# lightonai/fast-plaid

Measured on NVIDIA H100. Metric: queries/sec @ top_k=100, 1M-doc/128-dim index; MaxSim HBM GB/s vs roofline, higher is better.
Workload: dtype f16

## Files before the change

fast_plaid_b200/csrc/common.cuh:

```cuda
#pragma once

#include <cuda_fp16.h>
#include <cuda_runtime.h>
#include <stdint.h>

#include "../../include/fastplaid_b200.h"

struct WPerm {
  uint16_t v[16];
};

struct fpb_index {
  int device;
  int nbits;
  int dim;
  int pd;
  int sm_count;
  int64_t K;
  int64_t N;
  int64_t E;
  int64_t n_ivf;
  int64_t max_doc_len;
  int64_t doc_id_base;
  const __half* centroids;
  const int64_t* doc_offsets;
  const int32_t* doc_codes;
  const uint8_t* doc_residuals;
  const __half* token_norms;
  const int64_t* ivf_offsets;
  const int32_t* ivf_pids;
  WPerm w_perm;
  alignas(64) unsigned char tmap_centroids[128];
  int has_tmap;
};

void fpb_set_error(const char* fmt, ...);

#define FPB_CUDA_CHECK(expr)                                                              \
  do {                                                                                    \
    cudaError_t _e = (expr);                                                              \
    if (_e != cudaSuccess) {                                                              \
      fpb_set_error("%s failed: %s (%s:%d)", #expr, cudaGetErrorString(_e), __FILE__, __LINE__); \
      return FPB_ERR_CUDA;                                                                \
    }                                                                                     \
  } while (0)

#define FPB_LAUNCH_CHECK(name)                                                            \
  do {                                                                                    \
    cudaError_t _e = cudaGetLastError();                                                  \
    if (_e != cudaSuccess) {                                                              \
      fpb_set_error("launch of %s failed: %s", name, cudaGetErrorString(_e));            \
      return FPB_ERR_CUDA;                                                                \
    }                                                                                     \
  } while (0)

static inline int64_t fpb_align256(int64_t x) { return (x + 255) & ~int64_t(255); }
static inline int fpb_next_pow2(int x) {
  int p = 1;
  while (p < x) p <<= 1;
  return p;
}


__device__ __forceinline__ uint32_t f32_key(float f) {
  uint32_t u = __float_as_uint(f);
  if ((u << 1) == 0u) u = 0u;
  return (u & 0x80000000u) ? ~u : (u | 0x80000000u);
}
__device__ __forceinline__ float f32_unkey(uint32_t k) {
  uint32_t u = (k & 0x80000000u) ? (k & 0x7fffffffu) : ~k;
  return __uint_as_float(u);
}
__device__ __forceinline__ uint32_t f16_key(uint16_t h) {
  uint32_t u = h;
  if ((u & 0x7fffu) == 0u) u = 0u;
  return (u & 0x8000u) ? (~u & 0xffffu) : (u | 0x8000u);
}

__device__ __forceinline__ uint4 ldg_nc_na(const uint4* p) {
  uint4 r;
  asm volatile("ld.global.nc.L1::no_allocate.v4.u32 {%0,%1,%2,%3}, [%4];"
               : "=r"(r.x), "=r"(r.y), "=r"(r.z), "=r"(r.w)
               : "l"(p));
  return r;
}

__device__ __forceinline__ uint32_t smem_u32(const void* p) {
  return static_cast<uint32_t>(__cvta_generic_to_shared(p));
}

__device__ __forceinline__ void ldmatrix_x4(uint32_t& r0, uint32_t& r1, uint32_t& r2, uint32_t& r3,
                                            uint32_t addr) {
  asm volatile("ldmatrix.sync.aligned.m8n8.x4.shared.b16 {%0,%1,%2,%3}, [%4];"
               : "=r"(r0), "=r"(r1), "=r"(r2), "=r"(r3)
               : "r"(addr));
}

__device__ __forceinline__ void mma_16816(float (&c)[4], const uint32_t (&a)[4], uint32_t b0,
                                          uint32_t b1) {
  asm volatile(
      "mma.sync.aligned.m16n8k16.row.col.f32.f16.f16.f32 {%0,%1,%2,%3}, {%4,%5,%6,%7}, {%8,%9}, "
      "{%0,%1,%2,%3};"
      : "+f"(c[0]), "+f"(c[1]), "+f"(c[2]), "+f"(c[3])
      : "r"(a[0]), "r"(a[1]), "r"(a[2]), "r"(a[3]), "r"(b0), "r"(b1));
}

__device__ __forceinline__ uint32_t pack_half2_rn(float lo, float hi) {
  __half2 h = __floats2half2_rn(lo, hi);
  return *reinterpret_cast<uint32_t*>(&h);
}
__device__ __forceinline__ __half2 u32_as_half2(uint32_t u) { return *reinterpret_cast<__half2*>(&u); }
__device__ __forceinline__ uint32_t half2_as_u32(__half2 h) { return *reinterpret_cast<uint32_t*>(&h); }

#define FPB_PAD_SENTINEL (-10000.0f)
```

fast_plaid_b200/csrc/index.cu:

```cuda
#include <stdarg.h>
#include <stdio.h>
#include <string.h>

#include <cuda.h>

#include "kernels.h"

typedef CUresult (*fpb_encode_tiled_fn)(CUtensorMap*, CUtensorMapDataType, cuuint32_t, void*, const cuuint64_t*,
                                        const cuuint64_t*, const cuuint32_t*, const cuuint32_t*,
                                        CUtensorMapInterleave, CUtensorMapSwizzle, CUtensorMapL2promotion,
                                        CUtensorMapFloatOOBfill);

static int make_centroid_tmap(fpb_index* ix) {
  ix->has_tmap = 0;
  if (ix->dim != 128) return 0;
  void* fn = nullptr;
  cudaDriverEntryPointQueryResult qres;
  if (cudaGetDriverEntryPoint("cuTensorMapEncodeTiled", &fn, cudaEnableDefault, &qres) != cudaSuccess || !fn ||
      qres != cudaDriverEntryPointSuccess) {
    cudaGetLastError();
    return 0;
  }
  static_assert(sizeof(CUtensorMap) == 128, "CUtensorMap is 128 bytes");
  CUtensorMap* tm = reinterpret_cast<CUtensorMap*>(ix->tmap_centroids);
  const cuuint64_t gdim[2] = {cuuint64_t(ix->dim), cuuint64_t(ix->K)};
  const cuuint64_t gstride[1] = {cuuint64_t(ix->dim) * 2};
  const cuuint32_t box[2] = {64, 128};
  const cuuint32_t estr[2] = {1, 1};
  const CUresult r = reinterpret_cast<fpb_encode_tiled_fn>(fn)(
      tm, CU_TENSOR_MAP_DATA_TYPE_FLOAT16, 2, const_cast<__half*>(ix->centroids), gdim, gstride, box, estr,
      CU_TENSOR_MAP_INTERLEAVE_NONE, CU_TENSOR_MAP_SWIZZLE_128B, CU_TENSOR_MAP_L2_PROMOTION_L2_256B,
      CU_TENSOR_MAP_FLOAT_OOB_FILL_NONE);
  if (r == CUDA_SUCCESS) ix->has_tmap = 1;
  return 0;
}

static thread_local char g_err[512] = "";

void fpb_set_error(const char* fmt, ...) {
  va_list ap;
  va_start(ap, fmt);
  vsnprintf(g_err, sizeof(g_err), fmt, ap);
  va_end(ap);
}

extern "C" const char* fpb_last_error(void) { return g_err; }
extern "C" int fpb_abi_version(void) { return 6; }

static int bitrev(int x, int nbits) {
  int r = 0;
  for (int k = 0; k < nbits; ++k)
    if (x & (1 << k)) r |= 1 << (nbits - 1 - k);
  return r;
}

extern "C" int fpb_index_create(fpb_index** out, int device, int nbits, int dim, int64_t n_centroids,
                                const void* d_centroids, const void* d_bucket_weights,
                                int64_t n_docs, const int64_t* d_doc_offsets,
                                const int32_t* d_doc_codes, const uint8_t* d_doc_residuals, void* d_token_norms,
                                const int64_t* d_ivf_offsets, const int32_t* d_ivf_pids,
                                int64_t n_ivf, int64_t max_doc_len, int64_t doc_id_base) {
  if (!out) {
    fpb_set_error("fpb_index_create: out is NULL");
    return FPB_ERR_INVALID;
  }
  *out = nullptr;
  if (nbits != 2 && nbits != 4) {
    fpb_set_error("unsupported nbits=%d (2 and 4 are supported)", nbits);
    return FPB_ERR_UNSUPPORTED;
  }
  const int pd = dim * nbits / 8;
  if ((dim != 64 && dim != 128) || (pd != 16 && pd != 32 && pd != 64)) {
    fpb_set_error("unsupported embedding dim=%d with nbits=%d: this build supports dim 64 and 128", dim, nbits);
    return FPB_ERR_UNSUPPORTED;
  }
  if (n_centroids <= 0 || n_docs < 0 || !d_centroids || !d_bucket_weights || !d_doc_offsets) {
    fpb_set_error("fpb_index_create: bad sizes or NULL codec/offset pointers");
    return FPB_ERR_INVALID;
  }
  if (n_docs >= (int64_t(1) << 31) || n_centroids >= (int64_t(1) << 31)) {
    fpb_set_error("fpb_index_create: n_docs and n_centroids must fit in int32 per shard");
    return FPB_ERR_UNSUPPORTED;
  }
  FPB_CUDA_CHECK(cudaSetDevice(device));
  fpb_index* ix = new fpb_index();
  memset(ix, 0, sizeof(*ix));
  ix->device = device;
  ix->nbits = nbits;
  ix->dim = dim;
  ix->pd = pd;
  ix->K = n_centroids;
  ix->N = n_docs;
  ix->n_ivf = n_ivf;
  ix->max_doc_len = max_doc_len;
  ix->doc_id_base = doc_id_base;
  ix->centroids = static_cast<const __half*>(d_centroids);
  ix->doc_offsets = d_doc_offsets;
  ix->doc_codes = d_doc_codes;
  ix->doc_residuals = d_doc_residuals;
  ix->token_norms = static_cast<const __half*>(d_token_norms);
  ix->ivf_offsets = d_ivf_offsets;
  ix->ivf_pids = d_ivf_pids;
  cudaDeviceProp prop;
  cudaError_t e = cudaGetDeviceProperties(&prop, device);
  if (e != cudaSuccess) {
    delete ix;
    fpb_set_error("cudaGetDeviceProperties failed: %s", cudaGetErrorString(e));
    return FPB_ERR_CUDA;
  }
  ix->sm_count = prop.multiProcessorCount;
  uint16_t w[16];
  e = cudaMemcpy(w, d_bucket_weights, sizeof(uint16_t) * (1 << nbits), cudaMemcpyDeviceToHost);
  if (e != cudaSuccess) {
    delete ix;
    fpb_set_error("copy of bucket_weights failed: %s", cudaGetErrorString(e));
    return FPB_ERR_CUDA;
  }
  for (int i = 0; i < 16; ++i) ix->w_perm.v[i] = 0;
  for (int i = 0; i < (1 << nbits); ++i) ix->w_perm.v[i] = w[bitrev(i, nbits)];
  int64_t n_tokens = 0;
  if (n_docs > 0) {
    e = cudaMemcpy(&n_tokens, d_doc_offsets + n_docs, sizeof(int64_t), cudaMemcpyDeviceToHost);
    if (e != cudaSuccess) {
      delete ix;
      fpb_set_error("copy of doc_offsets[N] failed: %s", cudaGetErrorString(e));
      return FPB_ERR_CUDA;
    }
  }
  ix->E = n_tokens;
  if (n_tokens > 0 && !d_token_norms) {
    delete ix;
    fpb_set_error("fpb_index_create: d_token_norms (f16 [n_tokens], filled here) is NULL");
    return FPB_ERR_INVALID;
  }
  if (n_tokens > 0) {
    const int rc = launch_token_norms(ix, static_cast<__half*>(d_token_norms), nullptr);
    e = rc == FPB_OK ? cudaDeviceSynchronize() : cudaSuccess;
    if (rc != FPB_OK || e != cudaSuccess) {
      delete ix;
      if (rc == FPB_OK) fpb_set_error("token norm kernel failed: %s", cudaGetErrorString(e));
      return rc != FPB_OK ? rc : FPB_ERR_CUDA;
    }
  }
  make_centroid_tmap(ix);
  *out = ix;
  return FPB_OK;
}

extern "C" void fpb_index_destroy(fpb_index* index) { delete index; }

extern "C" int fpb_workspace_layout(const fpb_index* ix, int B, int Q, const fpb_params* p,
                                    fpb_layout* L) {
  if (!ix || !p || !L) {
    fpb_set_error("fpb_workspace_layout: NULL argument");
    return FPB_ERR_INVALID;
  }
  if (B <= 0 || Q <= 0) {
    fpb_set_error("fpb_workspace_layout: B=%d Q=%d must be positive", B, Q);
    return FPB_ERR_INVALID;
  }
  if (Q > 256) {
    fpb_set_error("queries with more than 256 tokens are not supported (Q=%d)", Q);
    return FPB_ERR_UNSUPPORTED;
  }
  if (p->n_ivf_probe < 1 || p->n_ivf_probe > 32) {
    fpb_set_error("n_ivf_probe=%d outside the supported range [1,32]", p->n_ivf_probe);
    return FPB_ERR_UNSUPPORTED;
  }
  if (p->n_full_scores < 1 || p->top_k < 1) {
    fpb_set_error("n_full_scores and top_k must be >= 1");
    return FPB_ERR_INVALID;
  }
  int R = p->n_full_scores / 4;
  if (R < 1) R = 1;
  if (R > 4096) {
    fpb_set_error("n_full_scores=%d: more than 4096 re-ranked documents per query is not supported",
                  p->n_full_scores);
    return FPB_ERR_UNSUPPORTED;
  }
  memset(L, 0, sizeof(*L));
  int Qp = fpb_next_pow2(Q < 16 ? 16 : Q);
  L->B = B;
  L->Q = Q;
  L->Qp = Qp;
  L->n_tiles = int((ix->K + 127) / 128);
  L->R = R;
  L->n_probe = p->n_ivf_probe;
  L->cand_cap = int(ix->N > 0 ? ix->N : 1);
  L->bitmap_words = int((ix->N + 31) / 32) + 1;
  int64_t off = 0;
  auto take = [&](int64_t bytes) {
    int64_t o = off;
    off += fpb_align256(bytes);
    return o;
  };
  L->off_queries = take(int64_t(B) * Qp * ix->dim * 2);
  L->off_S = take(int64_t(B) * ix->K * Qp * 2);
  L->off_tmax = take(int64_t(B) * Qp * L->n_tiles * 2);
  L->off_cells = take(int64_t(B) * Q * L->n_probe * 4);
  L->off_bitmap = take(int64_t(B) * L->bitmap_words * 4);
  L->off_n_cand = take(int64_t(B) * 4);
  L->off_cand = take(int64_t(B) * L->cand_cap * 4);
  L->off_approx = take(int64_t(B) * L->cand_cap * 4);
  L->off_work = take(int64_t(B + 8) * 4);
  L->off_n_rerank = take(int64_t(B) * 4);
  L->off_rerank = take(int64_t(B) * R * 4);
  L->off_rerank_approx = take(int64_t(B) * R * 4);
  L->off_exact = take(int64_t(B) * R * 4);
  const bool sub = (p->flags & FPB_FLAG_SUBSET) != 0;
  L->cbitmap_words = int((ix->K + 31) / 32) + 1;
  L->off_cbitmap = take(sub ? int64_t(B) * L->cbitmap_words * 4 : 0);
  L->off_clist = take(sub ? int64_t(B) * ix->K * 4 : 0);
  L->off_n_clist = take(sub ? int64_t(B) * 4 : 0);
  L->off_sbitmap = take(sub ? int64_t(B) * L->bitmap_words * 4 : 0);
  const bool direct = (p->flags & FPB_FLAG_APPROX_DIRECT) != 0;
  L->hb_words = int(((ix->K + 31) / 32 + 3) / 4 * 4);
  L->off_tau = take(direct ? 0 : int64_t(B) * Qp * 2);
  L->off_hibits = take(direct ? 0 : int64_t(B) * L->hb_words * 4);
  L->off_lb = take(direct ? 0 : int64_t(B) * L->cand_cap * 4);
  L->off_refine = take(direct ? 0 : int64_t(B) * L->cand_cap * 4);
  L->off_n_refine = take(int64_t(B) * 4);
  L->off_thresh = take(int64_t(B) * 4);
  L->off_work2 = take(int64_t(B + 8) * 4);
  L->off_stats = take(8 * 8);
  L->flags = p->flags;
  L->total_bytes = off;
  return FPB_OK;
}
```

fast_plaid_b200/csrc/k3_approx.cu:

```cuda
#include <math.h>
#include <stdlib.h>

#include "kernels.h"

namespace {

constexpr int64_t K3_TWO_PASS_MIN_TOKENS = 200000000;
constexpr int K3_THREADS = 256;
constexpr int K3_DOCS_PER_CHUNK = 64;
constexpr int K3A_DOCS_PER_CHUNK = 128;
constexpr int K3_WQ_FOR(int W, int FLUSH) { int n = 64; while (n < 32 * W + FLUSH) n <<= 1; return n; }

__global__ void k3_prefix_kernel(const int32_t* __restrict__ n_items, int B, int per_chunk,
                                 int32_t* __restrict__ work) {
  if (threadIdx.x == 0 && blockIdx.x == 0) {
    int acc = 0;
    for (int b = 0; b < B; ++b) {
      work[b] = acc;
      acc += (n_items[b] + per_chunk - 1) / per_chunk;
    }
    work[B] = acc;
    work[B + 1] = 0;
  }
}

__device__ __forceinline__ void k3_next_chunk(int32_t* work, int B, int* s_b, int* s_c) {
  __syncthreads();
  if (threadIdx.x == 0) {
    const int c = atomicAdd(&work[B + 1], 1);
    if (c >= work[B]) {
      *s_b = -1;
    } else {
      int lo = 0, hi = B - 1;
      while (lo < hi) {
        const int mid = (lo + hi + 1) >> 1;
        if (work[mid] <= c) lo = mid; else hi = mid - 1;
      }
      *s_b = lo;
      *s_c = c - work[lo];
    }
  }
  __syncthreads();
}

template <int LPR>
__device__ __forceinline__ void k3_reduce_groups(__half2& m0, __half2& m1, __half2& m2, __half2& m3) {
#pragma unroll
  for (int off = LPR; off < 32; off <<= 1) {
    m0 = __hmax2(m0, u32_as_half2(__shfl_xor_sync(0xffffffffu, half2_as_u32(m0), off)));
    m1 = __hmax2(m1, u32_as_half2(__shfl_xor_sync(0xffffffffu, half2_as_u32(m1), off)));
    m2 = __hmax2(m2, u32_as_half2(__shfl_xor_sync(0xffffffffu, half2_as_u32(m2), off)));
    m3 = __hmax2(m3, u32_as_half2(__shfl_xor_sync(0xffffffffu, half2_as_u32(m3), off)));
  }
}
template <int LPR, bool FULLQ = false>
__device__ __forceinline__ float k3_sum_columns(__half2 m0, __half2 m1, __half2 m2, __half2 m3, int col0, int Q) {
  float s = 0.f;
  const float2 f0 = __half22float2(m0), f1 = __half22float2(m1), f2 = __half22float2(m2), f3 = __half22float2(m3);
  if constexpr (FULLQ) {
    s += f0.x; s += f0.y; s += f1.x; s += f1.y; s += f2.x; s += f2.y; s += f3.x; s += f3.y;
#pragma unroll
    for (int off = 1; off < LPR; off <<= 1) s += __shfl_xor_sync(0xffffffffu, s, off);
    return s;
  }
  if (col0 + 0 < Q) s += f0.x;
  if (col0 + 1 < Q) s += f0.y;
  if (col0 + 2 < Q) s += f1.x;
  if (col0 + 3 < Q) s += f1.y;
  if (col0 + 4 < Q) s += f2.x;
  if (col0 + 5 < Q) s += f2.y;
  if (col0 + 6 < Q) s += f3.x;
  if (col0 + 7 < Q) s += f3.y;
#pragma unroll
  for (int off = 1; off < LPR; off <<= 1) s += __shfl_xor_sync(0xffffffffu, s, off);
  return s;
}

template <int LPR, int UNROLL, int MINB>
__global__ void __launch_bounds__(K3_THREADS, MINB)
k3_approx_kernel(const __half* __restrict__ S, int64_t K, int Q, const int64_t* __restrict__ doc_offsets,
                 const int32_t* __restrict__ codes, const int32_t* __restrict__ cand, int cand_cap,
                 const int32_t* __restrict__ n_cand, const int32_t* __restrict__ list,
                 const int32_t* __restrict__ n_list, int32_t* __restrict__ work, int B,
                 float* __restrict__ approx, unsigned long long* __restrict__ stats) {
  constexpr int QP = LPR * 8;
  constexpr int TPI = 32 / LPR;
  __shared__ int s_b, s_c;
  const int tid = threadIdx.x, lane = tid & 31, warp = tid >> 5;
  const int sub = lane % LPR, grp = lane / LPR;
  const __half2 sentinel = __float2half2_rn(FPB_PAD_SENTINEL);
  unsigned long long rows = 0;

  for (;;) {
    k3_next_chunk(work, B, &s_b, &s_c);
    const int b = s_b;
    if (b < 0) break;
    const int n = list ? n_list[b] : n_cand[b];
    const uint4* Sb = reinterpret_cast<const uint4*>(S + int64_t(b) * K * QP);
    const int32_t* cb = cand + int64_t(b) * cand_cap;
    const int32_t* lb = list ? list + int64_t(b) * cand_cap : nullptr;
    float* ab = approx + int64_t(b) * cand_cap;

    for (int i = 0; i < K3_DOCS_PER_CHUNK / 8; ++i) {
      const int j = s_c * K3_DOCS_PER_CHUNK + i * 8 + warp;
      if (j >= n) break;
      const int idx = lb ? lb[j] : j;
      const int d = cb[idx];
      const int64_t o0 = doc_offsets[d];
      const int len = int(doc_offsets[d + 1] - o0);
      rows += unsigned(len);
      __half2 m0 = sentinel, m1 = sentinel, m2 = sentinel, m3 = sentinel;
      for (int base = 0; base < len; base += 32 * UNROLL) {
        int code[UNROLL];
#pragma unroll
        for (int u = 0; u < UNROLL; ++u) {
          const int t = base + u * 32 + lane;
          code[u] = (t < len) ? __ldg(codes + o0 + t) : -1;
        }
#pragma unroll
        for (int u = 0; u < UNROLL; ++u) {
#pragma unroll
          for (int jj = 0; jj < LPR; ++jj) {
            const int c = __shfl_sync(0xffffffffu, code[u], jj * TPI + grp);
            if (c >= 0) {
              const uint4 v = __ldg(Sb + int64_t(c) * LPR + sub);
              m0 = __hmax2(m0, u32_as_half2(v.x));
              m1 = __hmax2(m1, u32_as_half2(v.y));
              m2 = __hmax2(m2, u32_as_half2(v.z));
              m3 = __hmax2(m3, u32_as_half2(v.w));
            }
          }
        }
      }
      k3_reduce_groups<LPR>(m0, m1, m2, m3);
      const float s = k3_sum_columns<LPR>(m0, m1, m2, m3, sub * 8, Q);
      if (lane == 0) ab[idx] = s;
    }
  }
  if (stats && lane == 0 && rows) atomicAdd(stats + 2, rows);
}

template <int LPR>
__device__ __forceinline__ void load_codes(int (&c)[LPR], const int32_t* p) {
  if constexpr (LPR == 2) {
    const int2 v = __ldg(reinterpret_cast<const int2*>(p));
    c[0] = v.x; c[1] = v.y;
  } else {
#pragma unroll
    for (int i = 0; i < LPR / 4; ++i) {
      const int4 v = __ldg(reinterpret_cast<const int4*>(p) + i);
      c[4 * i + 0] = v.x; c[4 * i + 1] = v.y; c[4 * i + 2] = v.z; c[4 * i + 3] = v.w;
    }
  }
}

template <int LPR, int UNROLL, int MINB>
__global__ void __launch_bounds__(K3_THREADS, MINB)
k3_approx_nsh_kernel(const __half* __restrict__ S, int64_t K, int Q, const int64_t* __restrict__ doc_offsets,
                     const int32_t* __restrict__ codes, int64_t n_codes, const int32_t* __restrict__ cand,
                     int cand_cap, const int32_t* __restrict__ n_cand, const int32_t* __restrict__ list,
                     const int32_t* __restrict__ n_list, int32_t* __restrict__ work, int B,
                     float* __restrict__ approx, unsigned long long* __restrict__ stats) {
  constexpr int QP = LPR * 8;
  __shared__ int s_b, s_c;
  const int tid = threadIdx.x, lane = tid & 31, warp = tid >> 5;
  const int sub = lane % LPR, grp = lane / LPR;
  const __half2 sentinel = __float2half2_rn(FPB_PAD_SENTINEL);
  unsigned long long rows = 0;

  for (;;) {
    k3_next_chunk(work, B, &s_b, &s_c);
    const int b = s_b;
    if (b < 0) break;
    const int n = list ? n_list[b] : n_cand[b];
    const uint4* Sb = reinterpret_cast<const uint4*>(S + int64_t(b) * K * QP) + sub;
    const int32_t* cb = cand + int64_t(b) * cand_cap;
    const int32_t* lb = list ? list + int64_t(b) * cand_cap : nullptr;
    float* ab = approx + int64_t(b) * cand_cap;

    for (int i = 0; i < K3_DOCS_PER_CHUNK / 8; ++i) {
      const int j = s_c * K3_DOCS_PER_CHUNK + i * 8 + warp;
      if (j >= n) break;
      const int idx = lb ? lb[j] : j;
      const int d = cb[idx];
      const int64_t o0 = doc_offsets[d];
      const int len = int(doc_offsets[d + 1] - o0);
      rows += unsigned(len);
      const int64_t w0 = o0 & ~int64_t(31);
      const int lo = int(o0 - w0), hi = lo + len;
      const int32_t* cw = codes + w0 + grp * LPR;
      const int64_t readable = n_codes - (w0 + grp * LPR);
      __half2 m0 = sentinel, m1 = sentinel, m2 = sentinel, m3 = sentinel;
      for (int f0 = 0; f0 < hi; f0 += 32 * UNROLL) {
        int c[UNROLL][LPR];
#pragma unroll
        for (int u = 0; u < UNROLL; ++u) {
          const int fo = f0 + u * 32;
          if (fo + LPR <= readable) {
            load_codes<LPR>(c[u], cw + fo);
          } else {
#pragma unroll
            for (int jj = 0; jj < LPR; ++jj) c[u][jj] = (fo + jj < readable) ? __ldg(cw + fo + jj) : 0;
          }
        }
#pragma unroll
        for (int u = 0; u < UNROLL; ++u) {
#pragma unroll
          for (int jj = 0; jj < LPR; ++jj) {
            const int f = f0 + u * 32 + grp * LPR + jj;
            if (unsigned(f - lo) < unsigned(len)) {
              const uint4 v = __ldg(Sb + int64_t(c[u][jj]) * LPR);
              m0 = __hmax2(m0, u32_as_half2(v.x));
              m1 = __hmax2(m1, u32_as_half2(v.y));
              m2 = __hmax2(m2, u32_as_half2(v.z));
              m3 = __hmax2(m3, u32_as_half2(v.w));
            }
          }
        }
      }
      k3_reduce_groups<LPR>(m0, m1, m2, m3);
      const float s = k3_sum_columns<LPR>(m0, m1, m2, m3, sub * 8, Q);
      if (lane == 0) ab[idx] = s;
    }
  }
  if (stats && lane == 0 && rows) atomicAdd(stats + 2, rows);
}

constexpr int K3_TAU_DOCS = 64;
constexpr int K3_TAU_THREADS = 1024;

template <int LPR>
__global__ void __launch_bounds__(K3_TAU_THREADS)
k3_tau_kernel(const __half* __restrict__ S, int64_t K, int Q, const int64_t* __restrict__ doc_offsets,
              const int32_t* __restrict__ codes, const int32_t* __restrict__ cand, int cand_cap,
              const int32_t* __restrict__ n_cand, const __half* __restrict__ tmax, int n_tiles, float lambda,
              __half* __restrict__ tau) {
  constexpr int QP = LPR * 8, TPI = 32 / LPR;
  constexpr int SUBS = LPR < 4 ? LPR : 4;
  __shared__ int hist[32][256];
  __shared__ int s_bin[32], s_rem[32];
  __shared__ uint32_t s_floor[32];
  __shared__ int s_redo;
  const int b = blockIdx.x, tid = threadIdx.x, lane = tid & 31, warp = tid >> 5;
  const int sub = lane % LPR, grp = lane / LPR;
  uint16_t* out = reinterpret_cast<uint16_t*>(tau) + int64_t(b) * QP;
  const int n = n_cand[b];
  const int ns = min(n, K3_TAU_DOCS);
  const int32_t* cb = cand + int64_t(b) * cand_cap;
  const uint4* Sb = reinterpret_cast<const uint4*>(S + int64_t(b) * K * QP);
  const int want = max(1, __float2int_rn(lambda * float(ns)));

  for (int g0 = 0; g0 < LPR; g0 += SUBS) {
    const bool mine = sub >= g0 && sub < g0 + SUBS;
    const int qrow = (sub - g0) * 8;
    __syncthreads();
    for (int col = warp; col < SUBS * 8; col += K3_TAU_THREADS / 32) {
      const int q = g0 * 8 + col;
      uint32_t mn = 0xffffu;
      if (q < Q) {
        const uint16_t* tm = reinterpret_cast<const uint16_t*>(tmax) + (int64_t(b) * QP + q) * n_tiles;
        for (int i = lane; i < n_tiles; i += 32) mn = min(mn, f16_key(tm[i]));
      }
#pragma unroll
      for (int off = 16; off > 0; off >>= 1) mn = min(mn, __shfl_xor_sync(0xffffffffu, mn, off));
      if (lane == 0) s_floor[col] = mn;
    }
    if (tid == 0) s_redo = 0;
    __syncthreads();
    for (int level = 0; level < 2; ++level) {
      for (int i = tid; i < 32 * 256; i += K3_TAU_THREADS) (&hist[0][0])[i] = 0;
      __syncthreads();
      uint32_t fl[8];
#pragma unroll
      for (int e = 0; e < 8; ++e) fl[e] = (mine && !s_redo) ? s_floor[qrow + e] : 0u;
      for (int j = warp; j < ns; j += K3_TAU_THREADS / 32) {
        const int d = cb[int64_t(j) * n / ns];
        const int64_t o0 = doc_offsets[d];
        const int len = int(doc_offsets[d + 1] - o0);
        for (int base = 0; base < len; base += 32) {
          const int t = base + lane;
          const int code = (t < len) ? __ldg(codes + o0 + t) : -1;
          constexpr int JB = LPR < 8 ? LPR : 8;
#pragma unroll 1
          for (int j0 = 0; j0 < LPR; j0 += JB) {
          uint4 vv[JB];
          int cc[JB];
#pragma unroll
          for (int jj = 0; jj < JB; ++jj) {
            cc[jj] = __shfl_sync(0xffffffffu, code, (j0 + jj) * TPI + grp);
            vv[jj] = make_uint4(0u, 0u, 0u, 0u);
            if (cc[jj] >= 0 && mine) vv[jj] = __ldg(Sb + int64_t(cc[jj]) * LPR + sub);
          }
#pragma unroll
          for (int jj = 0; jj < JB; ++jj) {
            const int c = cc[jj];
            if (c >= 0 && mine) {
              const uint4 v = vv[jj];
              const uint32_t w[4] = {v.x, v.y, v.z, v.w};
#pragma unroll
              for (int e = 0; e < 8; ++e) {
                const uint32_t key = f16_key(uint16_t(w[e >> 1] >> ((e & 1) * 16)));
                if (level == 0) {
                  if (key >= fl[e]) atomicAdd(&hist[qrow + e][key >> 8], 1);
                } else if (int(key >> 8) == s_bin[qrow + e]) {
                  atomicAdd(&hist[qrow + e][key & 255u], 1);
                }
              }
            }
          }
          }
        }
      }
      __syncthreads();
      if (tid < 32) {
        const int need = level == 0 ? want : s_rem[tid];
        int cum = 0, bin = 255;
        for (; bin > 0; --bin) {
          if (cum + hist[tid][bin] >= need) break;
          cum += hist[tid][bin];
        }
        if (level == 0) {
          s_bin[tid] = bin;
          s_rem[tid] = need - cum;
          if (bin == 0 && cum + hist[tid][0] < need && !s_redo && tid < SUBS * 8 && g0 * 8 + tid < Q &&
              s_floor[tid] != 0u)
            atomicExch(&s_redo, 2);
        } else {
          const int q = g0 * 8 + tid;
          if (q < QP) {
            uint32_t key = (uint32_t(s_bin[tid]) << 8) | uint32_t(bin);
            if (s_bin[tid] == 0 && bin == 0) key = f16_key(0xFC00u);
            uint16_t h = uint16_t((key & 0x8000u) ? (key & 0x7fffu) : (~key & 0xffffu));
            if (q >= Q) h = 0x7C00u;
            if (q < QP && tid < SUBS * 8) out[q] = h;
          }
        }
      }
      __syncthreads();
      if (level == 0 && s_redo == 2) {
        __syncthreads();
        if (tid == 0) s_redo = 1;
        __syncthreads();
        level = -1;
      }
    }
  }
}

template <int LPR>
__global__ void __launch_bounds__(256)
k3_hibits_kernel(const __half* __restrict__ S, int64_t K, const __half* __restrict__ tau,
                 uint32_t* __restrict__ hibits, int hb_words) {
  constexpr int QP = LPR * 8, TPI = 32 / LPR;
  const int b = blockIdx.y, lane = threadIdx.x & 31;
  const int64_t word = int64_t(blockIdx.x) * 8 + (threadIdx.x >> 5);
  const int64_t c0 = word * 32;
  if (c0 >= K) return;
  const int sub = lane % LPR, grp = lane / LPR;
  const uint4 t = *reinterpret_cast<const uint4*>(tau + int64_t(b) * QP + sub * 8);
  const uint4* Sb = reinterpret_cast<const uint4*>(S + int64_t(b) * K * QP);
  constexpr uint32_t GMASK = (LPR == 32) ? 0xffffffffu : ((1u << (LPR & 31)) - 1u);
  bool mine = false;
#pragma unroll
  for (int j = 0; j < LPR; ++j) {
    const int64_t c = c0 + j * TPI + grp;
    bool h = false;
    if (c < K) {
      const uint4 v = ldg_nc_na(Sb + c * LPR + sub);
      const unsigned any = __hge2_mask(u32_as_half2(v.x), u32_as_half2(t.x)) |
                           __hge2_mask(u32_as_half2(v.y), u32_as_half2(t.y)) |
                           __hge2_mask(u32_as_half2(v.z), u32_as_half2(t.z)) |
                           __hge2_mask(u32_as_half2(v.w), u32_as_half2(t.w));
      h = any != 0u;
    }
    const unsigned bal = __ballot_sync(0xffffffffu, h);
    if (lane / TPI == j) mine = ((bal >> ((lane % TPI) * LPR)) & GMASK) != 0u;
  }
  const unsigned w = __ballot_sync(0xffffffffu, mine);
  if (lane == 0) hibits[int64_t(b) * hb_words + word] = w;
}

__device__ __forceinline__ uint32_t k3_lds(uint32_t addr) {
  uint32_t v;
  asm volatile("ld.shared.u32 %0, [%1];" : "=r"(v) : "r"(addr));
  return v;
}
__device__ __forceinline__ unsigned k3_push(uint32_t word, uint32_t code, uint32_t ring_base, uint32_t ring_mask_bytes,
                                            uint32_t tail_bytes, uint32_t lt_mask) {
  unsigned mask;
  asm volatile(
      "{\n"
      ".reg .pred p;\n"
      ".reg .b32 t, r;\n"
      "shf.r.wrap.b32 t, %1, 0, %2;\n"
      "and.b32 t, t, 1;\n"
      "setp.ne.u32 p, t, 0;\n"
      "vote.sync.ballot.b32 %0, p, 0xffffffff;\n"
      "and.b32 r, %0, %6;\n"
      "popc.b32 r, r;\n"
      "shl.b32 r, r, 2;\n"
      "add.u32 r, r, %5;\n"
      "and.b32 r, r, %4;\n"
      "or.b32 r, r, %3;\n"
      "@p st.shared.u32 [r], %2;\n"
      "}"
      : "=r"(mask)
      : "r"(word), "r"(code), "r"(ring_base), "r"(ring_mask_bytes), "r"(tail_bytes), "r"(lt_mask)
      : "memory");
  return mask;
}

template <int LPR, int MINB, int W, int U, bool FULLQ, bool PAIR>
__global__ void __launch_bounds__(K3_THREADS, MINB)
k3_bound_kernel(const __half* __restrict__ S, int64_t K, int Q, const int64_t* __restrict__ doc_offsets,
                const int32_t* __restrict__ codes, const int32_t* __restrict__ cand, int cand_cap,
                const int32_t* __restrict__ n_cand, int32_t* __restrict__ work, int B,
                const __half* __restrict__ tau, const uint32_t* __restrict__ hibits, int hb_words,
                float* __restrict__ ub_out, float* __restrict__ lb_out, unsigned long long* __restrict__ stats) {
  constexpr int QP = LPR * 8;
  constexpr int TPI = 32 / LPR;
  constexpr int FLUSH = U * TPI;
  constexpr int DPW = K3A_DOCS_PER_CHUNK / (K3_THREADS / 32);
  constexpr int WQ = K3_WQ_FOR(W, FLUSH);
  static_assert(FLUSH + 32 * W <= WQ, "ring too small");
  extern __shared__ __align__(16) uint32_t k3_smem[];
  __shared__ int s_b, s_c;
  __shared__ int64_t s_o0[K3A_DOCS_PER_CHUNK];
  __shared__ int s_len[K3A_DOCS_PER_CHUNK];
  const int tid = threadIdx.x, lane = tid & 31, warp = tid >> 5;
  const int sub = lane % LPR, grp = lane / LPR;
  const uint32_t sb_bm = smem_u32(k3_smem);
  const uint32_t sb_wq = ((sb_bm + uint32_t(hb_words + 4) * 4u + (WQ * 4u - 1u)) & ~(WQ * 4u - 1u)) + uint32_t(warp) * (WQ * 4u);
  const int INV = hb_words * 32;
  unsigned lt_mask;
  asm("mov.u32 %0, %%lanemask_lt;" : "=r"(lt_mask));
  const __half2 sentinel = __float2half2_rn(FPB_PAD_SENTINEL);
  unsigned rows = 0, toks = 0;
  int cur_b = -1;
  if (tid < 4) k3_smem[hb_words + tid] = 0u;

  for (;;) {
    k3_next_chunk(work, B, &s_b, &s_c);
    const int b = s_b;
    if (b < 0) break;
    const int n = n_cand[b];
    const int32_t* cb = cand + int64_t(b) * cand_cap;
    if (tid < K3A_DOCS_PER_CHUNK) {
      const int idx = s_c * K3A_DOCS_PER_CHUNK + tid;
      int64_t o0 = 0;
      int len = -1;
      if (idx < n) {
        const int d = cb[idx];
        o0 = doc_offsets[d];
        len = int(doc_offsets[d + 1] - o0);
      }
      s_o0[tid] = o0;
      s_len[tid] = len;
    }
    if (b != cur_b) {
      const uint4* src = reinterpret_cast<const uint4*>(hibits + int64_t(b) * hb_words);
      for (int i = tid; i < hb_words / 4; i += K3_THREADS) reinterpret_cast<uint4*>(k3_smem)[i] = src[i];
      cur_b = b;
    }
    __syncthreads();
    const uint4* Sb = reinterpret_cast<const uint4*>(S + int64_t(b) * K * QP) + sub;
    const uint4* tqp = reinterpret_cast<const uint4*>(tau + int64_t(b) * QP + sub * 8);
    float* ub_chunk = ub_out + int64_t(b) * cand_cap + int64_t(s_c) * K3A_DOCS_PER_CHUNK;
    float* lb_chunk = lb_out + int64_t(b) * cand_cap + int64_t(s_c) * K3A_DOCS_PER_CHUNK;

    int slot = warp * DPW;
    const int slot_end = slot + DPW;
    int len = s_len[slot];
    if (len < 0) continue;
    int rel, left;
    const int32_t* cw;
    {
      const int64_t o0 = s_o0[slot];
      const int lo = int(o0 & 31);
      rel = lane - lo;
      left = (lo + len + 31) >> 5;
      cw = codes + (o0 - lo) + lane;
    }
    int c[W];
#pragma unroll
    for (int u = 0; u < W; ++u) {
      c[u] = INV;
      if (unsigned(rel + 32 * u) < unsigned(len)) c[u] = __ldg(cw + 32 * u);
    }
    uint32_t head = 0, tail = 0;
    __half2 m0 = sentinel, m1 = sentinel, m2 = sentinel, m3 = sentinel;
    __half2 a0 = sentinel, a1 = sentinel, a2 = sentinel, a3 = sentinel;
    int slot_a = -1;

    for (;;) {
      const bool last_of_doc = left <= W;
      int nlen = len, nrel = rel + 32 * W, nleft = left - W;
      const int32_t* ncw = cw + 32 * W;
      if (last_of_doc) {
        nlen = (slot + 1 < slot_end) ? s_len[slot + 1] : -1;
        if (nlen >= 0) {
          const int64_t o0 = s_o0[slot + 1];
          const int lo = int(o0 & 31);
          nrel = lane - lo;
          nleft = (lo + nlen + 31) >> 5;
          ncw = codes + (o0 - lo) + lane;
        }
      }
      int nx[W];
      {
        const unsigned nlen_u = nlen < 0 ? 0u : unsigned(nlen);
#pragma unroll
        for (int u = 0; u < W; ++u) {
          nx[u] = INV;
          if (unsigned(nrel + 32 * u) < nlen_u) nx[u] = __ldg(ncw + 32 * u);
        }
      }
      uint32_t wbit[W];
#pragma unroll
      for (int u = 0; u < W; ++u) wbit[u] = k3_lds(sb_bm + ((uint32_t(c[u]) >> 5) << 2));
#pragma unroll
      for (int u = 0; u < W; ++u) {
        const unsigned mask = k3_push(wbit[u], uint32_t(c[u]), sb_wq, WQ * 4u - 1u, tail << 2, lt_mask);
        tail += __popc(mask);
      }
      __syncwarp();
      while (tail - head >= FLUSH) {
        uint4 v[U];
#pragma unroll
        for (int k = 0; k < U; ++k) {
          const uint32_t code = k3_lds(sb_wq + (((head + k * TPI + grp) & (WQ - 1)) << 2));
          v[k] = __ldg(Sb + int64_t(code) * LPR);
        }
#pragma unroll
        for (int k = 0; k < U; ++k) {
          m0 = __hmax2(m0, u32_as_half2(v[k].x));
          m1 = __hmax2(m1, u32_as_half2(v[k].y));
          m2 = __hmax2(m2, u32_as_half2(v[k].z));
          m3 = __hmax2(m3, u32_as_half2(v[k].w));
        }
        head += FLUSH;
      }
      if (last_of_doc) {
        {
          const uint32_t rem = tail - head;
          uint4 v[U];
#pragma unroll
          for (int k = 0; k < U; ++k) {
            const uint32_t jj = k * TPI + grp;
            v[k] = make_uint4(half2_as_u32(sentinel), half2_as_u32(sentinel), half2_as_u32(sentinel),
                              half2_as_u32(sentinel));
            if (jj < rem) {
              const uint32_t code = k3_lds(sb_wq + (((head + jj) & (WQ - 1)) << 2));
              v[k] = __ldg(Sb + int64_t(code) * LPR);
            }
          }
#pragma unroll
          for (int k = 0; k < U; ++k) {
            m0 = __hmax2(m0, u32_as_half2(v[k].x));
            m1 = __hmax2(m1, u32_as_half2(v[k].y));
            m2 = __hmax2(m2, u32_as_half2(v[k].z));
            m3 = __hmax2(m3, u32_as_half2(v[k].w));
          }
        }
        rows += tail;
        toks += unsigned(len);
        const uint4 tq = __ldg(tqp);
        const int col0 = sub * 8;
        if (PAIR && LPR <= 8 && slot_a < 0 && nlen >= 0) {
          a0 = m0; a1 = m1; a2 = m2; a3 = m3;
          slot_a = slot;
        } else if (PAIR && LPR <= 8 && slot_a >= 0) {
          const bool up = lane >= 16;
          __half2 x0 = up ? m0 : a0, x1 = up ? m1 : a1, x2 = up ? m2 : a2, x3 = up ? m3 : a3;
          const __half2 y0 = up ? a0 : m0, y1 = up ? a1 : m1, y2 = up ? a2 : m2, y3 = up ? a3 : m3;
          x0 = __hmax2(x0, u32_as_half2(__shfl_xor_sync(0xffffffffu, half2_as_u32(y0), 16)));
          x1 = __hmax2(x1, u32_as_half2(__shfl_xor_sync(0xffffffffu, half2_as_u32(y1), 16)));
          x2 = __hmax2(x2, u32_as_half2(__shfl_xor_sync(0xffffffffu, half2_as_u32(y2), 16)));
          x3 = __hmax2(x3, u32_as_half2(__shfl_xor_sync(0xffffffffu, half2_as_u32(y3), 16)));
#pragma unroll
          for (int off = LPR; off < 16; off <<= 1) {
            x0 = __hmax2(x0, u32_as_half2(__shfl_xor_sync(0xffffffffu, half2_as_u32(x0), off)));
            x1 = __hmax2(x1, u32_as_half2(__shfl_xor_sync(0xffffffffu, half2_as_u32(x1), off)));
            x2 = __hmax2(x2, u32_as_half2(__shfl_xor_sync(0xffffffffu, half2_as_u32(x2), off)));
            x3 = __hmax2(x3, u32_as_half2(__shfl_xor_sync(0xffffffffu, half2_as_u32(x3), off)));
          }
          const float lb = k3_sum_columns<LPR, FULLQ>(x0, x1, x2, x3, col0, Q);
          const float ub = k3_sum_columns<LPR, FULLQ>(__hmax2(x0, u32_as_half2(tq.x)), __hmax2(x1, u32_as_half2(tq.y)),
                                                      __hmax2(x2, u32_as_half2(tq.z)), __hmax2(x3, u32_as_half2(tq.w)),
                                                      col0, Q);
          if ((lane & 15) == 0) {
            const int at = up ? slot : slot_a;
            ub_chunk[at] = ub;
            lb_chunk[at] = lb;
          }
          slot_a = -1;
        } else {
          k3_reduce_groups<LPR>(m0, m1, m2, m3);
          const float lb = k3_sum_columns<LPR, FULLQ>(m0, m1, m2, m3, col0, Q);
          const float ub = k3_sum_columns<LPR, FULLQ>(__hmax2(m0, u32_as_half2(tq.x)), __hmax2(m1, u32_as_half2(tq.y)),
                                                      __hmax2(m2, u32_as_half2(tq.z)), __hmax2(m3, u32_as_half2(tq.w)),
                                                      col0, Q);
          if (lane == 0) {
            ub_chunk[slot] = ub;
            lb_chunk[slot] = lb;
          }
        }
        if (nlen < 0) break;
        head = tail = 0;
        m0 = m1 = m2 = m3 = sentinel;
        ++slot;
      }
      __syncwarp();
#pragma unroll
      for (int u = 0; u < W; ++u) c[u] = nx[u];
      len = nlen;
      rel = nrel;
      left = nleft;
      cw = ncw;
    }
  }
  if (stats && lane == 0) {
    if (rows) atomicAdd(stats + 0, (unsigned long long)rows);
    if (toks) atomicAdd(stats + 1, (unsigned long long)toks);
  }
}

__device__ __forceinline__ void k3_find_bucket(const int* hist, int need, int lane, int* s_t, int* s_need) {
  int mine = 0;
  for (int k = 0; k < 64; ++k) mine += hist[lane * 64 + k];
  int above = 0;
  for (int l = 31; l >= 0; --l) {
    const int c = __shfl_sync(0xffffffffu, mine, l);
    if (l > lane) above += c;
  }
  if (above < need && above + mine >= need) {
    int cum = above, d = lane * 64 + 63;
    for (; d > lane * 64; --d) {
      const int h = hist[d];
      if (cum + h >= need) break;
      cum += h;
    }
    *s_t = d;
    *s_need = need - cum;
  }
}

__global__ void __launch_bounds__(1024)
k3_refine_list_kernel(const float* __restrict__ ub, const float* __restrict__ lb, int cand_cap,
                      const int32_t* __restrict__ n_cand, int n_dec, int refine_all, int32_t* __restrict__ list,
                      int32_t* __restrict__ n_list, float* __restrict__ thresh) {
  __shared__ int hist[2048];
  __shared__ float s_red[64];
  __shared__ int s_t, s_need, s_cnt;
  const int b = blockIdx.x, tid = threadIdx.x, lane = tid & 31;
  const int n = n_cand[b];
  const float* ubb = ub + int64_t(b) * cand_cap;
  const float* lbb = lb + int64_t(b) * cand_cap;
  int32_t* out = list + int64_t(b) * cand_cap;
  constexpr int FV = 8;
  float T = -INFINITY;
  if (!refine_all && n > n_dec) {
    float mn = INFINITY, mx = -INFINITY;
    for (int i0 = tid; i0 < n; i0 += 1024 * FV) {
      float v[FV];
#pragma unroll
      for (int u = 0; u < FV; ++u) v[u] = (i0 + u * 1024 < n) ? lbb[i0 + u * 1024] : NAN;
#pragma unroll
      for (int u = 0; u < FV; ++u) {
        mn = fminf(mn, v[u]);
        mx = fmaxf(mx, v[u]);
      }
    }
#pragma unroll
    for (int off = 16; off > 0; off >>= 1) {
      mn = fminf(mn, __shfl_xor_sync(0xffffffffu, mn, off));
      mx = fmaxf(mx, __shfl_xor_sync(0xffffffffu, mx, off));
    }
    if (lane == 0) {
      s_red[tid >> 5] = mn;
      s_red[32 + (tid >> 5)] = mx;
    }
    __syncthreads();
    mn = s_red[lane];
    mx = s_red[32 + lane];
#pragma unroll
    for (int off = 16; off > 0; off >>= 1) {
      mn = fminf(mn, __shfl_xor_sync(0xffffffffu, mn, off));
      mx = fmaxf(mx, __shfl_xor_sync(0xffffffffu, mx, off));
    }
    const float range = mx - mn;
    if (range > 0.f && range < 3.0e38f) {
      const float scale1 = 2047.0f / range;
      auto bucket1 = [&](float v) { return min(2047, max(0, __float2int_rz((v - mn) * scale1))); };
      for (int i = tid; i < 2048; i += 1024) hist[i] = 0;
      __syncthreads();
      for (int i0 = tid; i0 < n; i0 += 1024 * FV) {
        float v[FV];
#pragma unroll
        for (int u = 0; u < FV; ++u) v[u] = (i0 + u * 1024 < n) ? lbb[i0 + u * 1024] : 0.f;
#pragma unroll
        for (int u = 0; u < FV; ++u)
          if (i0 + u * 1024 < n && v[u] == v[u]) atomicAdd(&hist[bucket1(v[u])], 1);
      }
      if (tid == 0) s_t = -1;
      __syncthreads();
      if (tid < 32) k3_find_bucket(hist, n_dec, lane, &s_t, &s_need);
      __syncthreads();
      const int t1 = s_t, need1 = s_need;
      __syncthreads();
      if (t1 >= 0) {
        const float lo1 = mn + float(t1) / scale1;
        const float scale2 = 2047.0f * scale1;
        auto bucket2 = [&](float v) { return min(2047, max(0, __float2int_rz((v - lo1) * scale2))); };
        for (int i = tid; i < 2048; i += 1024) hist[i] = 0;
        __syncthreads();
        for (int i0 = tid; i0 < n; i0 += 1024 * FV) {
          float v[FV];
#pragma unroll
          for (int u = 0; u < FV; ++u) v[u] = (i0 + u * 1024 < n) ? lbb[i0 + u * 1024] : 0.f;
#pragma unroll
          for (int u = 0; u < FV; ++u)
            if (i0 + u * 1024 < n && v[u] == v[u] && bucket1(v[u]) == t1) atomicAdd(&hist[bucket2(v[u])], 1);
        }
        if (tid == 0) s_t = -1;
        __syncthreads();
        if (tid < 32) k3_find_bucket(hist, need1, lane, &s_t, &s_need);
        __syncthreads();
        const int t2 = s_t;
        float tmin = INFINITY;
        if (t2 >= 0) {
          for (int i0 = tid; i0 < n; i0 += 1024 * FV) {
            float v[FV];
#pragma unroll
            for (int u = 0; u < FV; ++u) v[u] = (i0 + u * 1024 < n) ? lbb[i0 + u * 1024] : NAN;
#pragma unroll
            for (int u = 0; u < FV; ++u) {
              if (v[u] == v[u]) {
                const int b1 = bucket1(v[u]);
                if (b1 > t1 || (b1 == t1 && bucket2(v[u]) >= t2)) tmin = fminf(tmin, v[u]);
              }
            }
          }
        }
#pragma unroll
        for (int off = 16; off > 0; off >>= 1) tmin = fminf(tmin, __shfl_xor_sync(0xffffffffu, tmin, off));
        __syncthreads();
        if (lane == 0) s_red[tid >> 5] = tmin;
        __syncthreads();
        tmin = s_red[lane];
#pragma unroll
        for (int off = 16; off > 0; off >>= 1) tmin = fminf(tmin, __shfl_xor_sync(0xffffffffu, tmin, off));
        if (t2 >= 0 && tmin < INFINITY) T = tmin;
      }
    } else if (range == 0.f) {
      T = mn;
    }
  }
  if (tid == 0) s_cnt = 0;
  __syncthreads();
  const int n_up = (n + 1023) / 1024 * 1024;
  for (int i = tid; i < n_up; i += 1024) {
    bool take = false;
    if (i < n) {
      const float u = ubb[i], l = lbb[i];
      take = (l < u) && (u >= T);
    }
    const unsigned m = __ballot_sync(0xffffffffu, take);
    int base = 0;
    if (lane == 0 && m) base = atomicAdd(&s_cnt, __popc(m));
    base = __shfl_sync(0xffffffffu, base, 0);
    if (take) out[base + __popc(m & ((1u << lane) - 1u))] = i;
  }
  __syncthreads();
  if (tid == 0) {
    n_list[b] = s_cnt;
    thresh[b] = T;
  }
}

__device__ __forceinline__ uint64_t approx_key(float a, uint32_t i) {
  return (uint64_t(f32_key(a)) << 32) | uint64_t(0xffffffffu - i);
}

__constant__ int K3B_LO[6] = {53, 42, 32, 21, 10, 0};
__constant__ int K3B_W[6] = {11, 11, 10, 11, 11, 10};
constexpr int K3B_VPT = 4;
constexpr int K3B_BCAP = 2048;

__global__ void __launch_bounds__(1024)
k3b_select_kernel(const float* __restrict__ approx, const int32_t* __restrict__ cand, int cand_cap,
                  const int32_t* __restrict__ n_cand, int n_dec, int Rp2, int32_t* __restrict__ rerank,
                  float* __restrict__ rerank_approx, int32_t* __restrict__ n_rerank) {
  extern __shared__ __align__(16) unsigned char smem_raw[];
  uint64_t* keys = reinterpret_cast<uint64_t*>(smem_raw);
  __shared__ int hist[2048];
  __shared__ int s_need, s_hd, s_cnt;
  __shared__ uint64_t s_prefix, s_mask;
  __shared__ uint64_t bkeys[K3B_BCAP];
  __shared__ float s_red[64];
  __shared__ int s_cnt2, s_fast;
  const int b = blockIdx.x, tid = threadIdx.x, lane = tid & 31;
  const int n = n_cand[b];
  const float* ab = approx + int64_t(b) * cand_cap;
  const int32_t* cb = cand + int64_t(b) * cand_cap;
  int32_t* rr = rerank + int64_t(b) * n_dec;
  float* ra = rerank_approx + int64_t(b) * n_dec;
  if (n <= n_dec) {
    for (int i = tid; i < n; i += 1024) {
      rr[i] = cb[i];
      ra[i] = ab[i];
    }
    if (tid == 0) n_rerank[b] = n;
    return;
  }
  {
    constexpr int FV = 8;
    float mn = INFINITY, mx = -INFINITY;
    for (int i0 = tid; i0 < n; i0 += 1024 * FV) {
      float v[FV];
#pragma unroll
      for (int u = 0; u < FV; ++u) v[u] = (i0 + u * 1024 < n) ? ab[i0 + u * 1024] : NAN;
#pragma unroll
      for (int u = 0; u < FV; ++u) {
        mn = fminf(mn, v[u]);
        mx = fmaxf(mx, v[u]);
      }
    }
#pragma unroll
    for (int off = 16; off > 0; off >>= 1) {
      mn = fminf(mn, __shfl_xor_sync(0xffffffffu, mn, off));
      mx = fmaxf(mx, __shfl_xor_sync(0xffffffffu, mx, off));
    }
    if (lane == 0) {
      s_red[tid >> 5] = mn;
      s_red[32 + (tid >> 5)] = mx;
    }
    for (int i = tid; i < 2048; i += 1024) hist[i] = 0;
    if (tid == 0) {
      s_cnt = 0;
      s_cnt2 = 0;
      s_fast = 0;
    }
    __syncthreads();
    mn = s_red[lane];
    mx = s_red[32 + lane];
#pragma unroll
    for (int off = 16; off > 0; off >>= 1) {
      mn = fminf(mn, __shfl_xor_sync(0xffffffffu, mn, off));
      mx = fmaxf(mx, __shfl_xor_sync(0xffffffffu, mx, off));
    }
    const float range = mx - mn;
    const bool usable = range > 0.f && range < 3.0e38f;
    const float scale = usable ? 2047.0f / range : 0.f;
    auto bucket = [&](float v) { return min(2047, max(0, __float2int_rz((v - mn) * scale))); };
    if (usable) {
      for (int i0 = tid; i0 < n; i0 += 1024 * FV) {
        float v[FV];
#pragma unroll
        for (int u = 0; u < FV; ++u) v[u] = (i0 + u * 1024 < n) ? ab[i0 + u * 1024] : 0.f;
#pragma unroll
        for (int u = 0; u < FV; ++u)
          if (i0 + u * 1024 < n) atomicAdd(&hist[bucket(v[u])], 1);
      }
      __syncthreads();
      if (tid < 32) {
        int mine = 0;
        for (int k = 0; k < 64; ++k) mine += hist[lane * 64 + k];
        int above = 0;
        for (int l = 31; l >= 0; --l) {
          const int c = __shfl_sync(0xffffffffu, mine, l);
          if (l > lane) above += c;
        }
        if (above < n_dec && above + mine >= n_dec) {
          int cum = above, d = lane * 64 + 63;
          for (; d > lane * 64; --d) {
            const int h = hist[d];
            if (cum + h >= n_dec) break;
            cum += h;
          }
          s_need = n_dec - cum;
          s_hd = d;
          s_fast = hist[d] <= K3B_BCAP ? 1 : 0;
        }
      }
      __syncthreads();
      if (s_fast) {
        const int t = s_hd;
        for (int i0 = tid; i0 < n; i0 += 1024 * FV) {
          float v[FV];
#pragma unroll
          for (int u = 0; u < FV; ++u) v[u] = (i0 + u * 1024 < n) ? ab[i0 + u * 1024] : 0.f;
#pragma unroll
          for (int u = 0; u < FV; ++u) {
            const int i = i0 + u * 1024;
            if (i < n) {
              const int bk = bucket(v[u]);
              if (bk > t) {
                keys[atomicAdd(&s_cnt, 1)] = approx_key(v[u], uint32_t(i));
              } else if (bk == t) {
                bkeys[atomicAdd(&s_cnt2, 1)] = approx_key(v[u], uint32_t(i));
              }
            }
          }
        }
        __syncthreads();
        const int c2 = s_cnt2, need2 = s_need;
        for (int i = c2 + tid; i < K3B_BCAP; i += 1024) bkeys[i] = 0ull;
        __syncthreads();
        for (int k = 2; k <= K3B_BCAP; k <<= 1) {
          for (int j = k >> 1; j > 0; j >>= 1) {
            for (int i = tid; i < K3B_BCAP; i += 1024) {
              const int ixj = i ^ j;
              if (ixj > i) {
                const bool up = (i & k) == 0;
                const uint64_t x = bkeys[i], y = bkeys[ixj];
                if ((x < y) == up) {
                  bkeys[i] = y;
                  bkeys[ixj] = x;
                }
              }
            }
            __syncthreads();
          }
        }
        const int c1 = s_cnt;
        for (int i = tid; i < need2; i += 1024) keys[c1 + i] = bkeys[i];
        __syncthreads();
        if (tid == 0) s_cnt = c1 + need2;
        __syncthreads();
      }
    }
  }
  const bool fast_done = s_fast != 0;
  if (!fast_done) {
  if (tid == 0) {
    s_need = n_dec;
    s_prefix = 0;
    s_mask = 0;
  }
  }
  const int stride = 1024 * K3B_VPT;
  const int n_up = (n + stride - 1) / stride * stride;
  if (!fast_done) {
  for (int pass = 0; pass < 6; ++pass) {
    const int lo = K3B_LO[pass], width = K3B_W[pass];
    const uint64_t dmask = (1ull << width) - 1ull;
    for (int i = tid; i < 2048; i += 1024) hist[i] = 0;
    __syncthreads();
    const uint64_t prefix = s_prefix, mask = s_mask;
    for (int i0 = tid; i0 < n_up; i0 += stride) {
      float v[K3B_VPT];
#pragma unroll
      for (int u = 0; u < K3B_VPT; ++u) {
        const int i = i0 + u * 1024;
        v[u] = (i < n) ? ab[i] : 0.f;
      }
#pragma unroll
      for (int u = 0; u < K3B_VPT; ++u) {
        const int i = i0 + u * 1024;
        const bool valid = i < n;
        const uint64_t key = valid ? approx_key(v[u], uint32_t(i)) : 0ull;
        const bool in = valid && ((key & mask) == prefix);
        const unsigned act = __ballot_sync(0xffffffffu, in);
        if (in) {
          const int bin = int((key >> lo) & dmask);
          const unsigned peers = __match_any_sync(act, bin);
          if (lane == __ffs(peers) - 1) atomicAdd(&hist[bin], __popc(peers));
        }
      }
    }
    __syncthreads();
    if (tid < 32) {
      const int nbins = 1 << width;
      const int per = nbins / 32;
      int mine = 0;
      for (int k = 0; k < per; ++k) mine += hist[lane * per + k];
      int above = 0;
      for (int l = 31; l >= 0; --l) {
        const int c = __shfl_sync(0xffffffffu, mine, l);
        if (l > lane) above += c;
      }
      const int need = s_need;
      const bool here = (above < need) && (above + mine >= need);
      if (here) {
        int cum = above, d = lane * per + per - 1;
        for (; d > lane * per; --d) {
          const int h = hist[d];
          if (cum + h >= need) break;
          cum += h;
        }
        s_need = need - cum;
        s_hd = hist[d];
        s_prefix = prefix | (uint64_t(d) << lo);
        s_mask = mask | (dmask << lo);
      }
    }
    __syncthreads();
    if (s_hd == s_need) break;
  }
  const uint64_t T = s_prefix;
  if (tid == 0) s_cnt = 0;
  __syncthreads();
  for (int i0 = tid; i0 < n_up; i0 += stride) {
    float v[K3B_VPT];
#pragma unroll
    for (int u = 0; u < K3B_VPT; ++u) {
      const int i = i0 + u * 1024;
      v[u] = (i < n) ? ab[i] : 0.f;
    }
#pragma unroll
    for (int u = 0; u < K3B_VPT; ++u) {
      const int i = i0 + u * 1024;
      if (i < n) {
        const uint64_t key = approx_key(v[u], uint32_t(i));
        if (key >= T) {
          const int pos = atomicAdd(&s_cnt, 1);
          if (pos < Rp2) keys[pos] = key;
        }
      }
    }
  }
  }
  __syncthreads();
  const int cnt = min(s_cnt, Rp2);
  for (int i = cnt + tid; i < Rp2; i += 1024) keys[i] = 0ull;
  __syncthreads();
  for (int k = 2; k <= Rp2; k <<= 1) {
    for (int j = k >> 1; j > 0; j >>= 1) {
      for (int i = tid; i < Rp2; i += 1024) {
        const int ixj = i ^ j;
        if (ixj > i) {
          const bool up = (i & k) == 0;
          const uint64_t x = keys[i], y = keys[ixj];
          if ((x < y) == up) {
            keys[i] = y;
            keys[ixj] = x;
          }
        }
      }
      __syncthreads();
    }
  }
  for (int r = tid; r < n_dec; r += 1024) {
    const uint32_t idx = 0xffffffffu - uint32_t(keys[r]);
    rr[r] = cb[idx];
    ra[r] = ab[idx];
  }
  if (tid == 0) n_rerank[b] = n_dec;
}

template <int LPR>
int launch_k3_exact(const fpb_index* ix, const Ws& ws, const int32_t* list, const int32_t* n_list, int32_t* work,
                    cudaStream_t st) {
  const fpb_layout& L = *ws.L;
  const int blocks = ix->sm_count * 8;
  if constexpr (LPR <= 4) {
    if ((reinterpret_cast<uintptr_t>(ix->doc_codes) & 15u) == 0) {
      k3_approx_nsh_kernel<LPR, 2, 6><<<blocks, K3_THREADS, 0, st>>>(
          ws.S(), ix->K, L.Q, ix->doc_offsets, ix->doc_codes, ix->E, ws.cand(), L.cand_cap, ws.n_cand(), list, n_list,
          work, L.B, ws.approx(), ws.stats());
      FPB_LAUNCH_CHECK("k3_approx_nsh");
      return FPB_OK;
    }
  }
  k3_approx_kernel<LPR, 2, 6><<<blocks, K3_THREADS, 0, st>>>(ws.S(), ix->K, L.Q, ix->doc_offsets, ix->doc_codes,
                                                             ws.cand(), L.cand_cap, ws.n_cand(), list, n_list, work,
                                                             L.B, ws.approx(), ws.stats());
  FPB_LAUNCH_CHECK("k3_approx");
  return FPB_OK;
}

float k3_tau_lambda(int Q) {
  static const float pinned = [] {
    const char* e = getenv("FPB_K3_LAMBDA");
    return e ? float(atof(e)) : 0.f;
  }();
  const float x = pinned > 0.f ? pinned : logf(float(Q < 2 ? 2 : Q)) - 1.45f;
  return x < 0.5f ? 0.5f : (x > 64.f ? 64.f : x);
}

template <int LPR>
int launch_k3_t(const fpb_index* ix, const Ws& ws, int flags, cudaStream_t st) {
  const fpb_layout& L = *ws.L;
  const bool forced = (flags & (FPB_FLAG_APPROX_TWO_PASS | FPB_FLAG_APPROX_EXACT_ALL)) != 0;
  const bool small_job = int64_t(L.B) * ix->E < K3_TWO_PASS_MIN_TOKENS;
  if ((flags & FPB_FLAG_APPROX_DIRECT) || size_t(L.hb_words) * 4 > 96 * 1024 || (!forced && small_job)) {
    FPB_CUDA_CHECK(cudaMemsetAsync(ws.n_refine(), 0, size_t(L.B) * 4, st));
    k3_prefix_kernel<<<1, 32, 0, st>>>(ws.n_cand(), L.B, K3_DOCS_PER_CHUNK, ws.work());
    FPB_LAUNCH_CHECK("k3_prefix");
    return launch_k3_exact<LPR>(ix, ws, nullptr, nullptr, ws.work(), st);
  }
  k3_tau_kernel<LPR><<<L.B, K3_TAU_THREADS, 0, st>>>(ws.S(), ix->K, L.Q, ix->doc_offsets, ix->doc_codes, ws.cand(),
                                                     L.cand_cap, ws.n_cand(), ws.tmax(), L.n_tiles, k3_tau_lambda(L.Q),
                                                     ws.tau());
  FPB_LAUNCH_CHECK("k3_tau");
  {
    dim3 grid(unsigned((ix->K + 255) / 256), unsigned(L.B));
    k3_hibits_kernel<LPR><<<grid, 256, 0, st>>>(ws.S(), ix->K, ws.tau(), ws.hibits(), L.hb_words);
    FPB_LAUNCH_CHECK("k3_hibits");
  }
  k3_prefix_kernel<<<1, 32, 0, st>>>(ws.n_cand(), L.B, K3A_DOCS_PER_CHUNK, ws.work());
  FPB_LAUNCH_CHECK("k3_prefix");
  {
    constexpr int TPI = 32 / LPR;
    constexpr int W = 6, U = 4, MINB = 4;
    const bool fullq = L.Q == L.Qp;
    auto kern = fullq ? k3_bound_kernel<LPR, MINB, W, U, true, true> : k3_bound_kernel<LPR, MINB, W, U, false, true>;
    const int minb = MINB, wq = K3_WQ_FOR(W, U * TPI);
    const size_t smem = size_t(L.hb_words + 4) * 4 + size_t(K3_THREADS / 32 + 1) * wq * 4;
    FPB_CUDA_CHECK(cudaFuncSetAttribute(kern, cudaFuncAttributeMaxDynamicSharedMemorySize, int(smem)));
    int per_sm = int((227 * 1024) / (smem + 1024 + 2048));
    per_sm = per_sm < 1 ? 1 : (per_sm > minb ? minb : per_sm);
    kern<<<ix->sm_count * per_sm, K3_THREADS, smem, st>>>(ws.S(), ix->K, L.Q, ix->doc_offsets, ix->doc_codes, ws.cand(),
                                                          L.cand_cap, ws.n_cand(), ws.work(), L.B, ws.tau(),
                                                          ws.hibits(), L.hb_words, ws.approx(), ws.lb(), ws.stats());
    FPB_LAUNCH_CHECK("k3_bound");
  }
  k3_refine_list_kernel<<<L.B, 1024, 0, st>>>(ws.approx(), ws.lb(), L.cand_cap, ws.n_cand(), L.R,
                                              (flags & FPB_FLAG_APPROX_EXACT_ALL) ? 1 : 0, ws.refine(), ws.n_refine(),
                                              ws.thresh());
  FPB_LAUNCH_CHECK("k3_refine_list");
  k3_prefix_kernel<<<1, 32, 0, st>>>(ws.n_refine(), L.B, K3_DOCS_PER_CHUNK, ws.work2());
  FPB_LAUNCH_CHECK("k3_prefix");
  return launch_k3_exact<LPR>(ix, ws, ws.refine(), ws.n_refine(), ws.work2(), st);
}

}

int launch_approx(const fpb_index* ix, const Ws& ws, int flags, cudaStream_t st) {
  const fpb_layout& L = *ws.L;
  switch (L.Qp / 8) {
    case 2: return launch_k3_t<2>(ix, ws, flags, st);
    case 4: return launch_k3_t<4>(ix, ws, flags, st);
    case 8: return launch_k3_t<8>(ix, ws, flags, st);
    case 16: return launch_k3_t<16>(ix, ws, flags, st);
    case 32: return launch_k3_t<32>(ix, ws, flags, st);
    default:
      fpb_set_error("approx scoring: unsupported padded query length %d", L.Qp);
      return FPB_ERR_UNSUPPORTED;
  }
}

int launch_select(const fpb_index* ix, const Ws& ws, cudaStream_t st) {
  (void)ix;
  const fpb_layout& L = *ws.L;
  const int Rp2 = fpb_next_pow2(L.R);
  FPB_CUDA_CHECK(cudaFuncSetAttribute(k3b_select_kernel, cudaFuncAttributeMaxDynamicSharedMemorySize, Rp2 * 8));
  k3b_select_kernel<<<L.B, 1024, size_t(Rp2) * 8, st>>>(ws.approx(), ws.cand(), L.cand_cap, ws.n_cand(),
                                                       L.R, Rp2, ws.rerank(), ws.rerank_approx(),
                                                       ws.n_rerank());
  FPB_LAUNCH_CHECK("k3b_select");
  return FPB_OK;
}
```

fast_plaid_b200/csrc/kernels.h:

```cpp
#pragma once
#include "common.cuh"

struct Ws {
  const fpb_layout* L;
  char* base;
  __half* queries() const { return reinterpret_cast<__half*>(base + L->off_queries); }
  __half* S() const { return reinterpret_cast<__half*>(base + L->off_S); }
  __half* tmax() const { return reinterpret_cast<__half*>(base + L->off_tmax); }
  int32_t* cells() const { return reinterpret_cast<int32_t*>(base + L->off_cells); }
  uint32_t* bitmap() const { return reinterpret_cast<uint32_t*>(base + L->off_bitmap); }
  int32_t* n_cand() const { return reinterpret_cast<int32_t*>(base + L->off_n_cand); }
  int32_t* cand() const { return reinterpret_cast<int32_t*>(base + L->off_cand); }
  float* approx() const { return reinterpret_cast<float*>(base + L->off_approx); }
  int32_t* work() const { return reinterpret_cast<int32_t*>(base + L->off_work); }
  int32_t* n_rerank() const { return reinterpret_cast<int32_t*>(base + L->off_n_rerank); }
  int32_t* rerank() const { return reinterpret_cast<int32_t*>(base + L->off_rerank); }
  float* rerank_approx() const { return reinterpret_cast<float*>(base + L->off_rerank_approx); }
  float* exact() const { return reinterpret_cast<float*>(base + L->off_exact); }
  uint32_t* cbitmap() const { return reinterpret_cast<uint32_t*>(base + L->off_cbitmap); }
  int32_t* clist() const { return reinterpret_cast<int32_t*>(base + L->off_clist); }
  int32_t* n_clist() const { return reinterpret_cast<int32_t*>(base + L->off_n_clist); }
  uint32_t* sbitmap() const { return reinterpret_cast<uint32_t*>(base + L->off_sbitmap); }
  __half* tau() const { return reinterpret_cast<__half*>(base + L->off_tau); }
  uint32_t* hibits() const { return reinterpret_cast<uint32_t*>(base + L->off_hibits); }
  float* lb() const { return reinterpret_cast<float*>(base + L->off_lb); }
  int32_t* refine() const { return reinterpret_cast<int32_t*>(base + L->off_refine); }
  int32_t* n_refine() const { return reinterpret_cast<int32_t*>(base + L->off_n_refine); }
  float* thresh() const { return reinterpret_cast<float*>(base + L->off_thresh); }
  int32_t* work2() const { return reinterpret_cast<int32_t*>(base + L->off_work2); }
  unsigned long long* stats() const { return reinterpret_cast<unsigned long long*>(base + L->off_stats); }
};

int launch_pad_queries(const fpb_index* ix, const Ws& ws, const __half* d_queries, cudaStream_t st);
int launch_centroid_scores(const fpb_index* ix, const Ws& ws, cudaStream_t st);
int launch_centroid_scores_v2(const fpb_index* ix, const Ws& ws, cudaStream_t st, bool* handled);
int launch_probe(const fpb_index* ix, const Ws& ws, bool subset, cudaStream_t st);
int launch_candidates(const fpb_index* ix, const Ws& ws, bool subset, cudaStream_t st);
int launch_subset_mark(const fpb_index* ix, const Ws& ws, const int32_t* d_ids, const int64_t* d_offsets,
                       int64_t max_len, cudaStream_t st);
int launch_subset_compact(const fpb_index* ix, const Ws& ws, cudaStream_t st);
int launch_subset_merge(const fpb_index* ix, const Ws& ws, const uint32_t* d_all, int n_shards, cudaStream_t st);
int launch_subset(const fpb_index* ix, const Ws& ws, const int32_t* d_ids, const int64_t* d_offsets,
                  int64_t max_len, cudaStream_t st);
int launch_compact(const uint32_t* bitmap, const uint32_t* mask, int words, int32_t* out, int cap, int32_t* n_out,
                   int B, cudaStream_t st);
int launch_approx(const fpb_index* ix, const Ws& ws, int flags, cudaStream_t st);
int launch_select(const fpb_index* ix, const Ws& ws, cudaStream_t st);
int launch_maxsim(const fpb_index* ix, const Ws& ws, cudaStream_t st);
int launch_token_norms(const fpb_index* ix, __half* d_out, cudaStream_t st);
int launch_maxsim_v4(const fpb_index* ix, const Ws& ws, cudaStream_t st, bool* handled);
int launch_maxsim_v5(const fpb_index* ix, const Ws& ws, cudaStream_t st, bool* handled);
int launch_rank(const fpb_index* ix, const Ws& ws, int top_k, int64_t* d_out_ids, float* d_out_scores,
                int32_t* d_out_counts, cudaStream_t st);
int launch_emit_keys(const fpb_index* ix, const Ws& ws, uint64_t* d_keys, cudaStream_t st);
int launch_apply_threshold(const Ws& ws, const uint64_t* d_all_keys, int n_shards, int rank, cudaStream_t st,
                           int b_stride = 0);
int launch_merge(const fpb_record* d_all_records, int n_shards, int b_stride, int n_queries, int R, int top_k,
                 int64_t* d_out_ids, float* d_out_scores, int32_t* d_out_counts, cudaStream_t stream);
int launch_emit_records(const fpb_index* ix, const Ws& ws, fpb_record* d_records, cudaStream_t st);

struct ExLayout {
  int B, Q, Qs, n_rows, top_k, grid;
  int64_t off_rows;
  int64_t off_acc;
  int64_t off_carry;
  int64_t off_counter;
  int64_t off_scores, off_cand, off_n_cand, off_n_rerank, off_rerank, off_rerank_approx;
  int64_t total_bytes;
};
int launch_exhaustive_scores(const fpb_index* ix, const ExLayout& X, char* ws, const __half* d_queries,
                             float* d_scores, cudaStream_t st);
```

fast_plaid_b200/engine.py:

```python

from __future__ import annotations

import contextlib
import ctypes
import dataclasses
import os
import threading
from typing import Any

import torch

_LIB_PATH = os.path.join(os.path.dirname(os.path.abspath(__file__)), "csrc", "libfastplaid_b200.so")
_lib = None
_lib_lock = threading.Lock()

FPB_OK = 0
FPB_ERR_INVALID = -1
FPB_ERR_CUDA = -2
FPB_ERR_UNSUPPORTED = -3
FPB_ERR_WORKSPACE = -4
FPB_ERR_NO_IVF = -5


class EngineUnavailableError(RuntimeError):
    """The CUDA extension is missing or unusable.  There is deliberately no fallback."""


class FpbParams(ctypes.Structure):
    _fields_ = [
        ("n_ivf_probe", ctypes.c_int32),
        ("n_full_scores", ctypes.c_int32),
        ("top_k", ctypes.c_int32),
        ("batch_size", ctypes.c_int32),
        ("flags", ctypes.c_int32),
    ]


FPB_FLAG_SUBSET = 1
FPB_FLAG_APPROX_EXACT_ALL = 2
FPB_FLAG_APPROX_DIRECT = 4
FPB_FLAG_APPROX_TWO_PASS = 8


class FpbLayout(ctypes.Structure):
    _fields_ = [
        ("total_bytes", ctypes.c_int64),
        ("B", ctypes.c_int32),
        ("Q", ctypes.c_int32),
        ("Qp", ctypes.c_int32),
        ("n_tiles", ctypes.c_int32),
        ("R", ctypes.c_int32),
        ("n_probe", ctypes.c_int32),
        ("cand_cap", ctypes.c_int32),
        ("bitmap_words", ctypes.c_int32),
        ("cbitmap_words", ctypes.c_int32),
        ("reserved0", ctypes.c_int32),
        ("off_queries", ctypes.c_int64),
        ("off_S", ctypes.c_int64),
        ("off_tmax", ctypes.c_int64),
        ("off_cells", ctypes.c_int64),
        ("off_bitmap", ctypes.c_int64),
        ("off_n_cand", ctypes.c_int64),
        ("off_cand", ctypes.c_int64),
        ("off_approx", ctypes.c_int64),
        ("off_work", ctypes.c_int64),
        ("off_n_rerank", ctypes.c_int64),
        ("off_rerank", ctypes.c_int64),
        ("off_rerank_approx", ctypes.c_int64),
        ("off_exact", ctypes.c_int64),
        ("off_cbitmap", ctypes.c_int64),
        ("off_clist", ctypes.c_int64),
        ("off_n_clist", ctypes.c_int64),
        ("off_sbitmap", ctypes.c_int64),
        ("off_tau", ctypes.c_int64),
        ("off_hibits", ctypes.c_int64),
        ("off_lb", ctypes.c_int64),
        ("off_refine", ctypes.c_int64),
        ("off_n_refine", ctypes.c_int64),
        ("off_thresh", ctypes.c_int64),
        ("off_work2", ctypes.c_int64),
        ("off_stats", ctypes.c_int64),
        ("hb_words", ctypes.c_int32),
        ("flags", ctypes.c_int32),
    ]


EXPORTED_SYMBOLS = [
    "fpb_last_error",
    "fpb_abi_version",
    "fpb_index_create",
    "fpb_index_destroy",
    "fpb_workspace_layout",
    "fpb_search_batch",
    "fpb_search_batch_subset",
    "fpb_search_batch_host",
    "fpb_stage_centroid_scores",
    "fpb_stage_subset",
    "fpb_stage_probe",
    "fpb_stage_candidates",
    "fpb_stage_approx",
    "fpb_stage_select",
    "fpb_stage_maxsim",
    "fpb_stage_rank",
    "fpb_stage_keys",
    "fpb_stage_records",
    "fpb_search_shard",
    "fpb_merge_shards",
    "fpb_shard_approx_keys",
    "fpb_shard_subset_begin",
    "fpb_shard_subset_keys",
    "fpb_shard_apply_threshold",
    "fpb_shard_exact_records",
    "fpb_comm_unique_id",
    "fpb_comm_create",
    "fpb_comm_destroy",
    "fpb_comm_nccl_version",
    "fpb_sharded_scratch_bytes",
    "fpb_search_batch_sharded",
    "fpb_search_batch_sharded_host",
    "fpb_exhaustive_workspace_bytes",
    "fpb_exhaustive_scores",
    "fpb_search_exhaustive",
    "fpb_reconstruct",
    "fpb_token_scores",
    "fpb_encode",
    "fpb_kmeans_assign",
    "fpb_kmeans_update",
    "fpb_cast_f32_to_f16_host",
    "fpb_cast_f32_to_f16_host_portable",
]


def library_path() -> str:
    return _LIB_PATH


def load_library() -> ctypes.CDLL:
    global _lib
    with _lib_lock:
        if _lib is not None:
            return _lib
        if not os.path.exists(_LIB_PATH):
            raise EngineUnavailableError(
                f"{_LIB_PATH} not found. Build it with `python -c 'import __graft_entry__ as g; g.build()'` "
                f"or `make -C fast_plaid_b200/csrc`. The engine has no CPU fallback."
            )
        lib = ctypes.CDLL(_LIB_PATH)
        vp, i32, i64, sz = ctypes.c_void_p, ctypes.c_int, ctypes.c_int64, ctypes.c_size_t
        lib.fpb_last_error.restype = ctypes.c_char_p
        lib.fpb_last_error.argtypes = []
        lib.fpb_abi_version.restype = i32
        lib.fpb_index_create.restype = i32
        lib.fpb_index_create.argtypes = [
            ctypes.POINTER(vp), i32, i32, i32, i64, vp, vp, i64, vp, vp, vp, vp, vp, vp, i64, i64, i64,
        ]
        lib.fpb_index_destroy.restype = None
        lib.fpb_index_destroy.argtypes = [vp]
        lib.fpb_workspace_layout.restype = i32
        lib.fpb_workspace_layout.argtypes = [vp, i32, i32, ctypes.POINTER(FpbParams), ctypes.POINTER(FpbLayout)]
        lib.fpb_search_batch.restype = i32
        lib.fpb_search_batch.argtypes = [vp, vp, i32, i32, ctypes.POINTER(FpbParams), vp, sz, vp, vp, vp, vp]
        lib.fpb_search_batch_subset.restype = i32
        lib.fpb_search_batch_subset.argtypes = [vp, vp, i32, i32, ctypes.POINTER(FpbParams), vp, vp, i64, vp, sz,
                                                vp, vp, vp, vp]
        lib.fpb_stage_subset.restype = i32
        lib.fpb_stage_subset.argtypes = [vp, vp, vp, i64, i32, i32, ctypes.POINTER(FpbParams), vp, sz, vp]
        lib.fpb_search_batch_host.restype = i32
        lib.fpb_search_batch_host.argtypes = [
            vp, vp, i32, i32, ctypes.POINTER(FpbParams), vp, sz, vp, vp, vp, vp, vp, vp, vp, vp,
        ]
        lib.fpb_stage_centroid_scores.restype = i32
        lib.fpb_stage_centroid_scores.argtypes = [vp, vp, i32, i32, ctypes.POINTER(FpbParams), vp, sz, vp]
        for name in ("fpb_stage_probe", "fpb_stage_candidates", "fpb_stage_approx", "fpb_stage_select",
                     "fpb_stage_maxsim"):
            fn = getattr(lib, name)
            fn.restype = i32
            fn.argtypes = [vp, i32, i32, ctypes.POINTER(FpbParams), vp, sz, vp]
        lib.fpb_stage_rank.restype = i32
        lib.fpb_stage_rank.argtypes = [vp, i32, i32, ctypes.POINTER(FpbParams), vp, sz, vp, vp, vp, vp]
        lib.fpb_stage_keys.restype = i32
        lib.fpb_stage_keys.argtypes = [vp, i32, i32, ctypes.POINTER(FpbParams), vp, sz, vp, vp]
        lib.fpb_stage_records.restype = i32
        lib.fpb_stage_records.argtypes = [vp, i32, i32, ctypes.POINTER(FpbParams), vp, sz, vp, vp]
        lib.fpb_search_shard.restype = i32
        lib.fpb_search_shard.argtypes = [vp, vp, i32, i32, ctypes.POINTER(FpbParams), vp, sz, vp, vp]
        lib.fpb_shard_approx_keys.restype = i32
        lib.fpb_shard_approx_keys.argtypes = [vp, vp, i32, i32, ctypes.POINTER(FpbParams), vp, sz, vp, vp]
        lib.fpb_shard_subset_begin.restype = i32
        lib.fpb_shard_subset_begin.argtypes = [vp, vp, i32, i32, ctypes.POINTER(FpbParams), vp, vp, i64, vp, sz, vp, vp]
        lib.fpb_shard_subset_keys.restype = i32
        lib.fpb_shard_subset_keys.argtypes = [vp, i32, i32, ctypes.POINTER(FpbParams), vp, sz, vp, i32, vp, vp]
        lib.fpb_shard_apply_threshold.restype = i32
        lib.fpb_shard_apply_threshold.argtypes = [vp, vp, i32, i32, i32, i32, ctypes.POINTER(FpbParams), vp, sz, vp]
        lib.fpb_shard_exact_records.restype = i32
        lib.fpb_shard_exact_records.argtypes = [vp, i32, i32, ctypes.POINTER(FpbParams), vp, sz, vp, vp]
        lib.fpb_comm_unique_id.restype = i32
        lib.fpb_comm_unique_id.argtypes = [vp]
        lib.fpb_comm_create.restype = i32
        lib.fpb_comm_create.argtypes = [ctypes.POINTER(vp), i32, i32, vp, i32]
        lib.fpb_comm_destroy.restype = None
        lib.fpb_comm_destroy.argtypes = [vp]
        lib.fpb_comm_nccl_version.restype = i32
        lib.fpb_sharded_scratch_bytes.restype = i64
        lib.fpb_sharded_scratch_bytes.argtypes = [i32, i32, i32]
        lib.fpb_search_batch_sharded.restype = i32
        lib.fpb_search_batch_sharded.argtypes = [vp, vp, i32, vp, i32, i32, ctypes.POINTER(FpbParams), vp, sz, vp, sz,
                                                 vp, vp, vp, vp]
        lib.fpb_search_batch_sharded_host.restype = i32
        lib.fpb_search_batch_sharded_host.argtypes = [vp, vp, i32, vp, i32, i32, ctypes.POINTER(FpbParams), vp, sz, vp,
                                                      sz, vp, vp, vp, vp, vp, vp, vp, vp]
        lib.fpb_merge_shards.restype = i32
        lib.fpb_merge_shards.argtypes = [vp, i32, i32, i32, i32, vp, vp, vp, vp]
        lib.fpb_reconstruct.restype = i32
        lib.fpb_reconstruct.argtypes = [vp, vp, i32, vp, vp, vp]
        for name in ("fpb_cast_f32_to_f16_host", "fpb_cast_f32_to_f16_host_portable"):
            fn = getattr(lib, name)
            fn.restype = i32
            fn.argtypes = [vp, vp, sz]
        lib.fpb_encode.restype = i32
        lib.fpb_encode.argtypes = [i32, i32, i32, i64, vp, vp, i64, vp, vp, vp, vp]
        lib.fpb_kmeans_assign.restype = i32
        lib.fpb_kmeans_assign.argtypes = [i32, i32, i64, vp, vp, vp, i64, vp, vp]
        lib.fpb_kmeans_update.restype = i32
        lib.fpb_kmeans_update.argtypes = [i32, i32, i64, vp, vp, vp, vp, vp, vp]
        lib.fpb_token_scores.restype = i32
        lib.fpb_token_scores.argtypes = [vp, vp, i32, vp, vp, i32, i64, vp, vp]
        lib.fpb_exhaustive_workspace_bytes.restype = i32
        lib.fpb_exhaustive_workspace_bytes.argtypes = [vp, i32, i32, i32, ctypes.POINTER(sz)]
        lib.fpb_exhaustive_scores.restype = i32
        lib.fpb_exhaustive_scores.argtypes = [vp, vp, i32, i32, vp, sz, vp, vp]
        lib.fpb_search_exhaustive.restype = i32
        lib.fpb_search_exhaustive.argtypes = [vp, vp, i32, i32, i32, vp, sz, vp, vp, vp, vp]
        _lib = lib
        return lib


def _check(rc: int) -> None:
    if rc == FPB_OK:
        return
    msg = load_library().fpb_last_error().decode("utf-8", "replace")
    if rc in (FPB_ERR_INVALID, FPB_ERR_NO_IVF, FPB_ERR_UNSUPPORTED):
        raise ValueError(msg)
    raise RuntimeError(msg)


def _require_cuda() -> None:
    if not torch.cuda.is_available():
        raise EngineUnavailableError(
            "fast_plaid_b200 needs a CUDA device (H100, sm_90a); there is no CPU search path."
        )


def check_supported(dim: int, nbits: int) -> None:
    if int(nbits) not in (2, 4):
        raise ValueError(f"unsupported nbits={nbits}: the engine supports nbits 2 and 4")
    if int(dim) not in (64, 128):
        raise ValueError(f"unsupported embedding dim={dim}: the engine supports dim 64 and 128")


def _ptr(t: torch.Tensor | None) -> int | None:
    return None if t is None else t.data_ptr()


@dataclasses.dataclass
class IndexTensors:

    nbits: int
    centroids: torch.Tensor
    bucket_weights: torch.Tensor
    doc_lengths: torch.Tensor
    doc_codes: torch.Tensor
    doc_residuals: torch.Tensor
    ivf: torch.Tensor | None
    ivf_lengths: torch.Tensor | None
    avg_residual: torch.Tensor | None = None
    bucket_cutoffs: torch.Tensor | None = None

    @property
    def num_documents(self) -> int:
        return int(self.doc_lengths.shape[0])

    @property
    def dim(self) -> int:
        return int(self.centroids.shape[1])


def encode_tokens(tokens: torch.Tensor, centroids: torch.Tensor, cutoffs: torch.Tensor,
                  nbits: int) -> tuple[torch.Tensor, torch.Tensor]:
    _require_cuda()
    lib = load_library()
    dev = tokens.device
    tokens = tokens.to(torch.float16).contiguous()
    centroids = centroids.to(dev, torch.float16).contiguous()
    cutoffs = cutoffs.to(dev, torch.float32).contiguous()
    n, dim = tokens.shape
    codes = torch.empty((n,), dtype=torch.int32, device=dev)
    res = torch.empty((n, dim * nbits // 8), dtype=torch.uint8, device=dev)
    with torch.cuda.device(dev):
        _check(lib.fpb_encode(dev.index, int(nbits), int(dim), int(centroids.shape[0]), centroids.data_ptr(),
                              tokens.data_ptr(), n, cutoffs.data_ptr(), codes.data_ptr(), res.data_ptr(),
                              torch.cuda.current_stream(dev).cuda_stream))
    return codes, res


def kmeans_assign(points: torch.Tensor, centroids: torch.Tensor) -> torch.Tensor:
    _require_cuda()
    lib = load_library()
    dev = points.device
    points = points.to(torch.float16).contiguous()
    centroids = centroids.to(dev, torch.float16).contiguous()
    bias = (-0.5 * (centroids.float() ** 2).sum(1)).contiguous()
    out = torch.empty((points.shape[0],), dtype=torch.int32, device=dev)
    with torch.cuda.device(dev):
        _check(lib.fpb_kmeans_assign(dev.index, int(points.shape[1]), int(centroids.shape[0]), centroids.data_ptr(),
                                     bias.data_ptr(), points.data_ptr(), int(points.shape[0]), out.data_ptr(),
                                     torch.cuda.current_stream(dev).cuda_stream))
    return out


def kmeans_update(points: torch.Tensor, assign: torch.Tensor, centroids: torch.Tensor) -> tuple[torch.Tensor, torch.Tensor]:
    _require_cuda()
    lib = load_library()
    dev = points.device
    K = int(centroids.shape[0])
    order = torch.argsort(assign.to(torch.int64), stable=True)
    counts = torch.bincount(assign.to(torch.int64), minlength=K)
    seg = torch.zeros(K + 1, dtype=torch.int64, device=dev)
    seg[1:] = counts.cumsum(0)
    shift = torch.zeros(K, dtype=torch.float32, device=dev)
    with torch.cuda.device(dev):
        _check(lib.fpb_kmeans_update(dev.index, int(points.shape[1]), K, points.data_ptr(), order.data_ptr(),
                                     seg.data_ptr(), centroids.data_ptr(), shift.data_ptr(),
                                     torch.cuda.current_stream(dev).cuda_stream))
    return counts, shift


def shard_tensors(data: IndexTensors, rank: int, world: int) -> tuple[IndexTensors, int]:
    n = data.num_documents
    lo = (n * rank) // world
    hi = (n * (rank + 1)) // world
    lens = data.doc_lengths.to(torch.int64).cpu()
    offs = torch.cat([torch.zeros(1, dtype=torch.int64), lens.cumsum(0)])
    t0, t1 = int(offs[lo]), int(offs[hi])
    ivf = ivf_lengths = None
    if data.ivf is not None:
        g_ivf = data.ivf.to(torch.int64).cpu()
        g_len = data.ivf_lengths.to(torch.int64).cpu()
        cell_of = torch.repeat_interleave(torch.arange(g_len.shape[0], dtype=torch.int64), g_len)
        keep = (g_ivf >= lo) & (g_ivf < hi)
        ivf = (g_ivf[keep] - lo).to(torch.int32)
        ivf_lengths = torch.bincount(cell_of[keep], minlength=g_len.shape[0]).to(torch.int64)
    shard = IndexTensors(
        nbits=data.nbits,
        centroids=data.centroids,
        bucket_weights=data.bucket_weights,
        doc_lengths=lens[lo:hi],
        doc_codes=data.doc_codes[t0:t1],
        doc_residuals=data.doc_residuals[t0:t1],
        ivf=ivf,
        ivf_lengths=ivf_lengths,
    )
    return shard, lo


UPLOAD_DIRECT_BYTES = 256 << 20
UPLOAD_CHUNK_BYTES = 64 << 20


def upload_narrow(src: torch.Tensor, device: torch.device, dtype: torch.dtype,
                  out: torch.Tensor | None = None) -> torch.Tensor:
    src = src if src.is_contiguous() else src.contiguous()
    out_bytes = src.numel() * torch.empty((), dtype=dtype).element_size()
    if src.device.type != "cpu" or out_bytes <= UPLOAD_DIRECT_BYTES or src.dim() == 0 or src.shape[0] == 0:
        if out is None:
            return src.to(device, dtype).contiguous()
        out.copy_(src.to(dtype) if src.device.type == "cpu" else src)
        return out
    if out is None:
        out = torch.empty(src.shape, dtype=dtype, device=device)
    row_bytes = max(1, out_bytes // src.shape[0])
    rows = max(1, UPLOAD_CHUNK_BYTES // row_bytes)
    stage = [torch.empty((rows,) + tuple(src.shape[1:]), dtype=dtype).pin_memory() for _ in range(2)]
    done = [torch.cuda.Event(), torch.cuda.Event()]
    copy_stream = torch.cuda.Stream(device=device)
    with torch.cuda.stream(copy_stream):
        for i, r0 in enumerate(range(0, src.shape[0], rows)):
            r1 = min(src.shape[0], r0 + rows)
            slot = i & 1
            if i >= 2:
                done[slot].synchronize()
            stage[slot][: r1 - r0].copy_(src[r0:r1])
            out[r0:r1].copy_(stage[slot][: r1 - r0], non_blocking=True)
            done[slot].record(copy_stream)
    copy_stream.synchronize()
    return out


FPB_COMM_ID_BYTES = 128


class ShardComm:

    def __init__(self, nranks: int, rank: int, unique_id: bytes, device: torch.device | str) -> None:
        _require_cuda()
        self._lib = load_library()
        self.device = torch.device(device)
        self.nranks, self.rank = int(nranks), int(rank)
        if len(unique_id) != FPB_COMM_ID_BYTES:
            raise ValueError("unique_id must be FPB_COMM_ID_BYTES bytes")
        buf = ctypes.create_string_buffer(bytes(unique_id), FPB_COMM_ID_BYTES)
        handle = ctypes.c_void_p()
        with torch.cuda.device(self.device):
            _check(self._lib.fpb_comm_create(ctypes.byref(handle), self.nranks, self.rank, buf, self.device.index))
        self._handle = handle

    @staticmethod
    def new_unique_id() -> bytes:
        buf = ctypes.create_string_buffer(FPB_COMM_ID_BYTES)
        _check(load_library().fpb_comm_unique_id(buf))
        return buf.raw

    @classmethod
    def from_process_group(cls, device: torch.device | str) -> "ShardComm":
        import torch.distributed as dist

        rank, world = dist.get_rank(), dist.get_world_size()
        box = [cls.new_unique_id() if rank == 0 else None]
        dist.broadcast_object_list(box, src=0)
        return cls(world, rank, box[0], device)

    def close(self) -> None:
        if getattr(self, "_handle", None) is not None and self._handle.value:
            self._lib.fpb_comm_destroy(self._handle)
            self._handle = ctypes.c_void_p()

    def __del__(self) -> None:
        try:
            self.close()
        except Exception:
            pass


def shard_grid(rank: int, world: int, n_query_groups: int) -> tuple[int, int, int]:
    if n_query_groups < 1 or world % n_query_groups != 0:
        raise ValueError(f"{n_query_groups} query groups do not divide {world} ranks")
    n_shards = world // n_query_groups
    return rank // n_shards, rank % n_shards, n_shards


class DeviceIndex:

    def __init__(self, data: IndexTensors, device: str | torch.device, doc_id_base: int = 0) -> None:
        _require_cuda()
        self._lib = load_library()
        self.device = torch.device(device)
        if self.device.type != "cuda":
            raise ValueError(f"Unsupported device string: '{device}' (the engine runs on CUDA only)")
        if self.device.index is None:
            self.device = torch.device("cuda", torch.cuda.current_device())
        dev = self.device
        self.nbits = int(data.nbits)
        self.dim = data.dim
        self.doc_id_base = int(doc_id_base)
        with torch.cuda.device(dev):
            self.centroids = data.centroids.to(dev, torch.float16).contiguous()
            self.bucket_weights = data.bucket_weights.to(dev, torch.float16).contiguous()
            lens = data.doc_lengths.to(torch.int64)
            self.num_documents = int(lens.shape[0])
            self.max_doc_len = int(lens.max()) if self.num_documents > 0 else 0
            offs = torch.zeros(self.num_documents + 1, dtype=torch.int64)
            offs[1:] = lens.cpu().cumsum(0)
            self.num_tokens = int(offs[-1])
            self.doc_offsets = offs.to(dev)
            self.doc_codes = upload_narrow(data.doc_codes[: self.num_tokens], dev, torch.int32)
            self.doc_residuals = upload_narrow(data.doc_residuals[: self.num_tokens], dev, torch.uint8)
            if self.doc_codes.numel() == 0:
                self.doc_codes = torch.zeros(1, dtype=torch.int32, device=dev)
                self.doc_residuals = torch.zeros((1, self.dim * self.nbits // 8), dtype=torch.uint8, device=dev)
            self.num_centroids = int(self.centroids.shape[0])
            if data.ivf is not None and data.ivf_lengths is not None:
                il = data.ivf_lengths.to(torch.int64).cpu()
                if il.shape[0] < self.num_centroids:
                    il = torch.cat([il, torch.zeros(self.num_centroids - il.shape[0], dtype=torch.int64)])
                io = torch.zeros(il.shape[0] + 1, dtype=torch.int64)
                io[1:] = il.cumsum(0)
                self.ivf_offsets = io.to(dev)
                self.ivf_pids = upload_narrow(data.ivf, dev, torch.int32)
                if self.ivf_pids.numel() == 0:
                    self.ivf_pids = torch.zeros(1, dtype=torch.int32, device=dev)
                n_ivf = int(io[-1])
            else:
                self.ivf_offsets = None
                self.ivf_pids = None
                n_ivf = 0
            self.token_norms = torch.empty(max(self.num_tokens, 1), dtype=torch.float16, device=dev)
            handle = ctypes.c_void_p()
            _check(
                self._lib.fpb_index_create(
                    ctypes.byref(handle), dev.index, self.nbits, self.dim, self.num_centroids,
                    _ptr(self.centroids), _ptr(self.bucket_weights), self.num_documents,
                    _ptr(self.doc_offsets), _ptr(self.doc_codes), _ptr(self.doc_residuals), _ptr(self.token_norms),
                    _ptr(self.ivf_offsets), _ptr(self.ivf_pids), n_ivf, self.max_doc_len, self.doc_id_base,
                )
            )
        self._handle = handle
        self._ws: dict[tuple, FpbLayout] = {}
        self._buf: torch.Tensor | None = None
        self._io: dict[tuple, dict[str, torch.Tensor]] = {}
        self._lock = threading.Lock()
        self._search_lock = threading.RLock()
        self._last_stream: torch.cuda.Stream | None = None
        self._approx_direct = False
        self._approx_calls = 0
        self._approx_hold = 0

    @contextlib.contextmanager
    def _exclusive(self):
        with self._search_lock:
            if getattr(self, "_handle", None) is None or not self._handle.value:
                raise RuntimeError("this DeviceIndex has been closed")
            st = torch.cuda.current_stream(self.device)
            if self._last_stream is not None and self._last_stream != st:
                st.wait_stream(self._last_stream)
            self._last_stream = st
            yield

    def close(self) -> None:
        lock = getattr(self, "_search_lock", None)
        with (lock if lock is not None else contextlib.nullcontext()):
            if getattr(self, "_handle", None) is not None and self._handle.value:
                try:
                    torch.cuda.synchronize(self.device)
                except Exception:
                    pass
                self._lib.fpb_index_destroy(self._handle)
                self._handle = ctypes.c_void_p()
            self._ws = {}
            self._buf = None
            self._io = {}

    def __del__(self) -> None:
        try:
            self.close()
        except Exception:
            pass

    @property
    def has_ivf(self) -> bool:
        return self.ivf_offsets is not None

    @staticmethod
    def make_params(top_k: int, n_full_scores: int, n_ivf_probe: int, batch_size: int = 2000,
                    flags: int = 0) -> FpbParams:
        return FpbParams(int(n_ivf_probe), int(n_full_scores), int(top_k), int(batch_size), int(flags))

    @staticmethod
    def with_flags(params: FpbParams, flags: int) -> FpbParams:
        return FpbParams(params.n_ivf_probe, params.n_full_scores, params.top_k, params.batch_size,
                         params.flags | int(flags))

    @staticmethod
    def with_subset_flag(params: FpbParams) -> FpbParams:
        return FpbParams(params.n_ivf_probe, params.n_full_scores, params.top_k, params.batch_size,
                         params.flags | FPB_FLAG_SUBSET)

    def layout(self, B: int, Q: int, params: FpbParams) -> FpbLayout:
        lay = FpbLayout()
        _check(self._lib.fpb_workspace_layout(self._handle, B, Q, ctypes.byref(params), ctypes.byref(lay)))
        return lay

    def workspace(self, B: int, Q: int, params: FpbParams) -> tuple[torch.Tensor, FpbLayout]:
        key = (B, Q, params.n_ivf_probe, params.n_full_scores, params.top_k, params.flags)
        with self._lock:
            lay = self._ws.get(key)
            if lay is None:
                lay = self.layout(B, Q, params)
                if len(self._ws) > 64:
                    self._ws.clear()
                self._ws[key] = lay
            need = int(lay.total_bytes)
            if self._buf is None or self._buf.numel() < need:
                self._buf = None
                self._buf = torch.empty(need, dtype=torch.uint8, device=self.device)
            return self._buf, lay

    def max_queries_per_call(self, Q: int, params: FpbParams, budget_bytes: int = 6 << 30) -> int:
        key = ("maxq", Q, params.n_ivf_probe, params.n_full_scores, params.top_k, params.flags, budget_bytes)
        hit = self._ws.get(key)
        if hit is not None:
            return hit
        val = self._max_queries_per_call(Q, params, budget_bytes)
        self._ws[key] = val
        return val

    def _max_queries_per_call(self, Q: int, params: FpbParams, budget_bytes: int) -> int:
        one = self.layout(1, Q, params).total_bytes
        two = self.layout(2, Q, params).total_bytes
        per_q = max(1, two - one)
        return max(1, int((budget_bytes - one) // per_q) + 1)

    def _stream(self) -> int:
        return torch.cuda.current_stream(self.device).cuda_stream

    def _subset_csr(self, subset: list[list[int]], s: int, e: int) -> tuple[torch.Tensor, torch.Tensor, int]:
        lens = [len(x) for x in subset[s:e]]
        offs = torch.zeros(len(lens) + 1, dtype=torch.int64)
        offs[1:] = torch.tensor(lens, dtype=torch.int64).cumsum(0)
        flat = [i for x in subset[s:e] for i in x]
        ids = torch.tensor(flat if flat else [0], dtype=torch.int64)
        ids = ids.clamp(-1, 2**31 - 1).to(torch.int32)
        return ids.to(self.device), offs.to(self.device), (max(lens) if lens else 0)

    def search(
        self, queries: torch.Tensor, params: FpbParams, subset: list[list[int]] | None = None
    ) -> tuple[torch.Tensor, torch.Tensor, torch.Tensor]:
        if queries.dim() != 3:
            raise ValueError(f"Expected a 3D tensor for queries, but got shape {list(queries.shape)}")
        if queries.dtype != torch.float16 or queries.device != self.device:
            raise ValueError("DeviceIndex.search expects fp16 queries on the index device")
        queries = queries.contiguous()
        B, Q, D = queries.shape
        if D != self.dim:
            raise ValueError(f"query dim {D} != index dim {self.dim}")
        k = params.top_k
        ids = torch.empty((B, k), dtype=torch.int64, device=self.device)
        scores = torch.empty((B, k), dtype=torch.float32, device=self.device)
        counts = torch.empty((B,), dtype=torch.int32, device=self.device)
        if B == 0:
            return ids, scores, counts
        if subset is not None:
            if len(subset) != B:
                raise ValueError("Subset length must match number of queries.")
            params = FpbParams(params.n_ivf_probe, params.n_full_scores, params.top_k, params.batch_size,
                               params.flags | FPB_FLAG_SUBSET)
        step = self.max_queries_per_call(Q, params)
        with self._exclusive(), torch.cuda.device(self.device):
            for s in range(0, B, step):
                e = min(B, s + step)
                buf, lay = self.workspace(e - s, Q, params)
                if subset is None:
                    _check(
                        self._lib.fpb_search_batch(
                            self._handle, queries[s:e].data_ptr(), e - s, Q, ctypes.byref(params), buf.data_ptr(),
                            buf.numel(), ids[s:e].data_ptr(), scores[s:e].data_ptr(), counts[s:e].data_ptr(),
                            self._stream(),
                        )
                    )
                else:
                    sid, soff, smax = self._subset_csr(subset, s, e)
                    _check(
                        self._lib.fpb_search_batch_subset(
                            self._handle, queries[s:e].data_ptr(), e - s, Q, ctypes.byref(params), sid.data_ptr(),
                            soff.data_ptr(), smax, buf.data_ptr(), buf.numel(), ids[s:e].data_ptr(),
                            scores[s:e].data_ptr(), counts[s:e].data_ptr(), self._stream(),
                        )
                    )
                    self._keepalive = (sid, soff)
        return ids, scores, counts

    def exhaustive_workspace_bytes(self, B: int, Q: int, top_k: int) -> int:
        out = ctypes.c_size_t()
        _check(self._lib.fpb_exhaustive_workspace_bytes(self._handle, B, Q, top_k, ctypes.byref(out)))
        return int(out.value)

    def _exhaustive_buffer(self, nbytes: int) -> torch.Tensor:
        with self._lock:
            if self._buf is None or self._buf.numel() < nbytes:
                self._buf = None
                self._buf = torch.empty(nbytes, dtype=torch.uint8, device=self.device)
            return self._buf

    def _check_queries(self, queries: torch.Tensor) -> torch.Tensor:
        if queries.dim() != 3:
            raise ValueError(f"Expected a 3D tensor for queries, but got shape {list(queries.shape)}")
        if queries.dtype != torch.float16 or queries.device != self.device:
            raise ValueError("DeviceIndex expects fp16 queries on the index device")
        if queries.shape[2] != self.dim:
            raise ValueError(f"query dim {queries.shape[2]} != index dim {self.dim}")
        return queries.contiguous()

    def _exhaustive_step(self, B: int, Q: int, top_k: int, budget_bytes: int) -> int:
        if self.exhaustive_workspace_bytes(B, Q, top_k) <= budget_bytes:
            return B
        lo, hi = 1, B
        while lo < hi:
            mid = (lo + hi + 1) // 2
            if self.exhaustive_workspace_bytes(mid, Q, top_k) <= budget_bytes:
                lo = mid
            else:
                hi = mid - 1
        return lo

    def exhaustive_scores(self, queries: torch.Tensor) -> torch.Tensor:
        queries = self._check_queries(queries)
        B, Q, _ = queries.shape
        scores = torch.empty((B, self.num_documents), dtype=torch.float32, device=self.device)
        if B == 0:
            return scores
        with self._exclusive(), torch.cuda.device(self.device):
            buf = self._exhaustive_buffer(self.exhaustive_workspace_bytes(B, Q, 0))
            _check(
                self._lib.fpb_exhaustive_scores(
                    self._handle, queries.data_ptr(), B, Q, buf.data_ptr(), buf.numel(), scores.data_ptr(),
                    self._stream(),
                )
            )
        return scores

    def search_exhaustive(self, queries: torch.Tensor, top_k: int, budget_bytes: int = 6 << 30
                          ) -> tuple[torch.Tensor, torch.Tensor, torch.Tensor]:
        queries = self._check_queries(queries)
        B, Q, _ = queries.shape
        k = int(top_k)
        ids = torch.empty((B, k), dtype=torch.int64, device=self.device)
        scores = torch.empty((B, k), dtype=torch.float32, device=self.device)
        counts = torch.empty((B,), dtype=torch.int32, device=self.device)
        if B == 0:
            return ids, scores, counts
        step = self._exhaustive_step(B, Q, k, budget_bytes)
        with self._exclusive(), torch.cuda.device(self.device):
            for s in range(0, B, step):
                e = min(B, s + step)
                buf = self._exhaustive_buffer(self.exhaustive_workspace_bytes(e - s, Q, k))
                _check(
                    self._lib.fpb_search_exhaustive(
                        self._handle, queries[s:e].data_ptr(), e - s, Q, k, buf.data_ptr(), buf.numel(),
                        ids[s:e].data_ptr(), scores[s:e].data_ptr(), counts[s:e].data_ptr(), self._stream(),
                    )
                )
        return ids, scores, counts

    def _host_io(self, B: int, Q: int, k: int) -> dict[str, torch.Tensor]:
        key = (B, Q, k)
        with self._lock:
            io = self._io.get(key)
            if io is None:
                while len(self._io) >= 4:
                    self._io.pop(next(iter(self._io)))
                D = self.dim
                io = {
                    "d_q": torch.empty((B, Q, D), dtype=torch.float16, device=self.device),
                    "d_ids": torch.empty((B, k), dtype=torch.int64, device=self.device),
                    "d_scores": torch.empty((B, k), dtype=torch.float32, device=self.device),
                    "d_counts": torch.empty((B,), dtype=torch.int32, device=self.device),
                    "h_q": torch.empty((B, Q, D), dtype=torch.float16).pin_memory(),
                    "h_ids": torch.empty((B, k), dtype=torch.int64).pin_memory(),
                    "h_scores": torch.empty((B, k), dtype=torch.float32).pin_memory(),
                    "h_counts": torch.empty((B,), dtype=torch.int32).pin_memory(),
                }
                self._io[key] = io
        return io

    def _cast_into_pinned(self, queries_host: torch.Tensor, h_q: torch.Tensor) -> None:
        if queries_host.dtype == torch.float32 and queries_host.is_contiguous():
            _check(self._lib.fpb_cast_f32_to_f16_host(queries_host.data_ptr(), h_q.data_ptr(), queries_host.numel()))
        else:
            h_q.copy_(queries_host)

    def stage_queries(self, queries_host: torch.Tensor, top_k: int) -> torch.Tensor:
        B, Q, _ = queries_host.shape
        io = self._host_io(B, Q, top_k)
        self._cast_into_pinned(queries_host, io["h_q"])
        io["d_q"].copy_(io["h_q"], non_blocking=True)
        return io["d_q"]

    def search_host(
        self, queries_host: torch.Tensor, params: FpbParams
    ) -> tuple[torch.Tensor, torch.Tensor, torch.Tensor]:
        if queries_host.dim() != 3:
            raise ValueError(f"Expected a 3D tensor for queries, but got shape {list(queries_host.shape)}")
        if queries_host.device.type != "cpu" or not queries_host.dtype.is_floating_point:
            raise ValueError("search_host expects floating-point queries in host memory")
        B, Q, D = queries_host.shape
        if D != self.dim:
            raise ValueError(f"query dim {D} != index dim {self.dim}")
        if B == 0:
            k = params.top_k
            return (torch.empty((0, k), dtype=torch.int64), torch.empty((0, k), dtype=torch.float32),
                    torch.empty((0,), dtype=torch.int32))
        with self._exclusive(), torch.cuda.device(self.device):
            params = self._approx_flags(params)
            step = self.max_queries_per_call(Q, params)
            io = self._host_io(B, Q, params.top_k)
            self._cast_into_pinned(queries_host, io["h_q"])
            queries_host = io["h_q"]
            for s in range(0, B, step):
                e = min(B, s + step)
                buf, lay = self.workspace(e - s, Q, params)
                _check(
                    self._lib.fpb_search_batch_host(
                        self._handle, queries_host[s:e].data_ptr(), e - s, Q, ctypes.byref(params),
                        buf.data_ptr(), buf.numel(), io["d_q"][s:e].data_ptr(), io["d_ids"][s:e].data_ptr(),
                        io["d_scores"][s:e].data_ptr(), io["d_counts"][s:e].data_ptr(),
                        io["h_ids"][s:e].data_ptr(), io["h_scores"][s:e].data_ptr(),
                        io["h_counts"][s:e].data_ptr(), self._stream(),
                    )
                )
            self._adapt_approx_mode(buf, lay)
            return io["h_ids"].clone(), io["h_scores"].clone(), io["h_counts"].clone()

    def search_records(self, queries: torch.Tensor, params: FpbParams) -> torch.Tensor:
        queries = queries.contiguous()
        B, Q, _ = queries.shape
        buf, lay = self.workspace(B, Q, params)
        rec = torch.empty((B, lay.R, 16), dtype=torch.uint8, device=self.device)
        with self._exclusive(), torch.cuda.device(self.device):
            _check(
                self._lib.fpb_search_shard(
                    self._handle, queries.data_ptr(), B, Q, ctypes.byref(params), buf.data_ptr(), buf.numel(),
                    rec.data_ptr(), self._stream(),
                )
            )
        return rec

    APPROX_PROBE_EVERY = 8
    APPROX_DIRECT_ABOVE = 0.30
    APPROX_HOLD_CALLS = 64

    def _approx_flags(self, params: FpbParams) -> FpbParams:
        if self._approx_direct and not (params.flags & (FPB_FLAG_APPROX_EXACT_ALL | FPB_FLAG_APPROX_DIRECT |
                                                        FPB_FLAG_APPROX_TWO_PASS)):
            return self.with_flags(params, FPB_FLAG_APPROX_DIRECT)
        return params

    def _adapt_approx_mode(self, buf: torch.Tensor, lay: FpbLayout) -> None:
        if self._approx_direct:
            self._approx_hold -= 1
            if self._approx_hold <= 0:
                self._approx_direct = False
            return
        self._approx_calls += 1
        if self._approx_calls % self.APPROX_PROBE_EVERY or lay.flags & FPB_FLAG_APPROX_DIRECT:
            return
        v = self.views(buf, lay)
        both = torch.stack([v["n_refine"].sum(), v["n_cand"].sum()]).cpu()
        n_ref, n_cand = int(both[0]), int(both[1])
        if n_cand > 0 and n_ref / n_cand > self.APPROX_DIRECT_ABOVE:
            self._approx_direct = True
            self._approx_hold = self.APPROX_HOLD_CALLS

    def _sharded_io(self, comm: ShardComm, n_query_groups: int, B: int, Q: int, params: FpbParams):
        b_local = -(-B // n_query_groups)
        buf, lay = self.workspace(b_local, Q, params)
        need = int(self._lib.fpb_sharded_scratch_bytes(b_local, lay.R, comm.nranks))
        if getattr(self, "_scratch", None) is None or self._scratch.numel() < need:
            self._scratch = torch.empty(need, dtype=torch.uint8, device=self.device)
        return buf, self._scratch

    def search_sharded(self, comm: ShardComm, n_query_groups: int, queries: torch.Tensor,
                       params: FpbParams) -> tuple[torch.Tensor, torch.Tensor, torch.Tensor]:
        queries = queries.contiguous()
        B, Q, _ = queries.shape
        k = params.top_k
        ids = torch.empty((B, k), dtype=torch.int64, device=self.device)
        scores = torch.empty((B, k), dtype=torch.float32, device=self.device)
        counts = torch.empty((B,), dtype=torch.int32, device=self.device)
        with self._exclusive(), torch.cuda.device(self.device):
            buf, scratch = self._sharded_io(comm, n_query_groups, B, Q, params)
            _check(self._lib.fpb_search_batch_sharded(
                self._handle, comm._handle, n_query_groups, queries.data_ptr(), B, Q, ctypes.byref(params),
                buf.data_ptr(), buf.numel(), scratch.data_ptr(), scratch.numel(), ids.data_ptr(), scores.data_ptr(),
                counts.data_ptr(), self._stream()))
        return ids, scores, counts

    def search_sharded_host(self, comm: ShardComm, n_query_groups: int, queries_host: torch.Tensor,
                            params: FpbParams) -> tuple[torch.Tensor, torch.Tensor, torch.Tensor]:
        B, Q, D = queries_host.shape
        if D != self.dim:
            raise ValueError(f"query dim {D} != index dim {self.dim}")
        with self._exclusive(), torch.cuda.device(self.device):
            io = self._host_io(B, Q, params.top_k)
            self._cast_into_pinned(queries_host, io["h_q"])
            buf, scratch = self._sharded_io(comm, n_query_groups, B, Q, params)
            _check(self._lib.fpb_search_batch_sharded_host(
                self._handle, comm._handle, n_query_groups, io["h_q"].data_ptr(), B, Q, ctypes.byref(params),
                buf.data_ptr(), buf.numel(), scratch.data_ptr(), scratch.numel(), io["d_q"].data_ptr(),
                io["d_ids"].data_ptr(), io["d_scores"].data_ptr(), io["d_counts"].data_ptr(), io["h_ids"].data_ptr(),
                io["h_scores"].data_ptr(), io["h_counts"].data_ptr(), self._stream()))
            return io["h_ids"].clone(), io["h_scores"].clone(), io["h_counts"].clone()

    def shard_approx_keys(self, queries: torch.Tensor, params: FpbParams) -> torch.Tensor:
        queries = queries.contiguous()
        B, Q, _ = queries.shape
        buf, lay = self.workspace(B, Q, params)
        keys = torch.empty((B, lay.R), dtype=torch.int64, device=self.device)
        with self._exclusive(), torch.cuda.device(self.device):
            _check(self._lib.fpb_shard_approx_keys(self._handle, queries.data_ptr(), B, Q, ctypes.byref(params),
                                                   buf.data_ptr(), buf.numel(), keys.data_ptr(), self._stream()))
        return keys

    def shard_subset_begin(self, queries: torch.Tensor, params: FpbParams, subset: list[list[int]]) -> torch.Tensor:
        queries = queries.contiguous()
        B, Q, _ = queries.shape
        buf, lay = self.workspace(B, Q, params)
        sid, soff, smax = self._subset_csr(subset, 0, B)
        cb = torch.empty((B, lay.cbitmap_words), dtype=torch.int32, device=self.device)
        with self._exclusive(), torch.cuda.device(self.device):
            _check(self._lib.fpb_shard_subset_begin(self._handle, queries.data_ptr(), B, Q, ctypes.byref(params),
                                                    sid.data_ptr(), soff.data_ptr(), smax, buf.data_ptr(),
                                                    buf.numel(), cb.data_ptr(), self._stream()))
            torch.cuda.current_stream(self.device).synchronize()
        return cb

    def shard_subset_keys(self, all_cbitmaps: torch.Tensor, Q: int, params: FpbParams) -> torch.Tensor:
        n_shards, B, _ = all_cbitmaps.shape
        buf, lay = self.workspace(B, Q, params)
        keys = torch.empty((B, lay.R), dtype=torch.int64, device=self.device)
        with self._exclusive(), torch.cuda.device(self.device):
            _check(self._lib.fpb_shard_subset_keys(self._handle, B, Q, ctypes.byref(params), buf.data_ptr(),
                                                   buf.numel(), all_cbitmaps.contiguous().data_ptr(), n_shards,
                                                   keys.data_ptr(), self._stream()))
        return keys

    def shard_exact_records(self, all_keys: torch.Tensor, rank: int, Q: int, params: FpbParams) -> torch.Tensor:
        n_shards, B, R = all_keys.shape
        buf, lay = self.workspace(B, Q, params)
        rec = torch.empty((B, R, 16), dtype=torch.uint8, device=self.device)
        with self._exclusive(), torch.cuda.device(self.device):
            _check(self._lib.fpb_shard_apply_threshold(self._handle, all_keys.contiguous().data_ptr(), n_shards, rank,
                                                       B, Q, ctypes.byref(params), buf.data_ptr(), buf.numel(),
                                                       self._stream()))
            _check(self._lib.fpb_shard_exact_records(self._handle, B, Q, ctypes.byref(params), buf.data_ptr(),
                                                     buf.numel(), rec.data_ptr(), self._stream()))
        return rec

    def merge_records(
        self, all_records: torch.Tensor, top_k: int
    ) -> tuple[torch.Tensor, torch.Tensor, torch.Tensor]:
        n_shards, B, R, _ = all_records.shape
        ids = torch.empty((B, top_k), dtype=torch.int64, device=self.device)
        scores = torch.empty((B, top_k), dtype=torch.float32, device=self.device)
        counts = torch.empty((B,), dtype=torch.int32, device=self.device)
        with self._exclusive(), torch.cuda.device(self.device):
            _check(
                self._lib.fpb_merge_shards(
                    all_records.contiguous().data_ptr(), n_shards, B, R, top_k, ids.data_ptr(),
                    scores.data_ptr(), counts.data_ptr(), self._stream(),
                )
            )
        return ids, scores, counts

    def run_stages(self, queries: torch.Tensor, params: FpbParams, upto: str = "rank",
                   subset: list[list[int]] | None = None) -> dict[str, Any]:
        order = ["centroid_scores", "probe", "candidates", "approx", "select", "maxsim", "rank"]
        if subset is not None:
            params = FpbParams(params.n_ivf_probe, params.n_full_scores, params.top_k, params.batch_size,
                               params.flags | FPB_FLAG_SUBSET)
            order.insert(1, "subset")
        queries = queries.contiguous()
        B, Q, _ = queries.shape
        buf, lay = self.workspace(B, Q, params)
        st = self._stream()
        p = ctypes.byref(params)
        out: dict[str, Any] = {"layout": lay, "workspace": buf}
        with self._exclusive(), torch.cuda.device(self.device):
            for name in order:
                if name == "centroid_scores":
                    _check(self._lib.fpb_stage_centroid_scores(self._handle, queries.data_ptr(), B, Q, p,
                                                               buf.data_ptr(), buf.numel(), st))
                elif name == "subset":
                    sid, soff, smax = self._subset_csr(subset, 0, B)
                    _check(self._lib.fpb_stage_subset(self._handle, sid.data_ptr(), soff.data_ptr(), smax, B, Q, p,
                                                      buf.data_ptr(), buf.numel(), st))
                    torch.cuda.synchronize(self.device)
                elif name == "rank":
                    k = params.top_k
                    ids = torch.empty((B, k), dtype=torch.int64, device=self.device)
                    scores = torch.empty((B, k), dtype=torch.float32, device=self.device)
                    counts = torch.empty((B,), dtype=torch.int32, device=self.device)
                    _check(self._lib.fpb_stage_rank(self._handle, B, Q, p, buf.data_ptr(), buf.numel(),
                                                    ids.data_ptr(), scores.data_ptr(), counts.data_ptr(), st))
                    out.update(ids=ids, scores=scores, counts=counts)
                else:
                    fn = getattr(self._lib, f"fpb_stage_{name}")
                    _check(fn(self._handle, B, Q, p, buf.data_ptr(), buf.numel(), st))
                if name == upto:
                    break
        out.update(self.views(buf, lay))
        return out

    def stage_fn(self, name: str, queries: torch.Tensor, params: FpbParams):
        queries = queries.contiguous()
        B, Q, _ = queries.shape
        buf, lay = self.workspace(B, Q, params)
        p = ctypes.byref(params)
        st = self._stream()
        if name == "centroid_scores":
            return lambda: _check(self._lib.fpb_stage_centroid_scores(
                self._handle, queries.data_ptr(), B, Q, p, buf.data_ptr(), buf.numel(), st))
        fn = getattr(self._lib, f"fpb_stage_{name}")
        return lambda: _check(fn(self._handle, B, Q, p, buf.data_ptr(), buf.numel(), st))

    def views(self, buf: torch.Tensor, lay: FpbLayout) -> dict[str, torch.Tensor]:
        B, Q, Qp, R = lay.B, lay.Q, lay.Qp, lay.R
        K = self.num_centroids

        def v(off: int, nbytes: int, dtype: torch.dtype, shape: tuple) -> torch.Tensor:
            return buf[off : off + nbytes].view(dtype).view(*shape)

        return {
            "S": v(lay.off_S, B * K * Qp * 2, torch.float16, (B, K, Qp)),
            "tmax": v(lay.off_tmax, B * Qp * lay.n_tiles * 2, torch.float16, (B, Qp, lay.n_tiles)),
            "cells": v(lay.off_cells, B * Q * lay.n_probe * 4, torch.int32, (B, Q, lay.n_probe)),
            "n_cand": v(lay.off_n_cand, B * 4, torch.int32, (B,)),
            "cand": v(lay.off_cand, B * lay.cand_cap * 4, torch.int32, (B, lay.cand_cap)),
            "approx": v(lay.off_approx, B * lay.cand_cap * 4, torch.float32, (B, lay.cand_cap)),
            "n_rerank": v(lay.off_n_rerank, B * 4, torch.int32, (B,)),
            "rerank": v(lay.off_rerank, B * R * 4, torch.int32, (B, R)),
            "rerank_approx": v(lay.off_rerank_approx, B * R * 4, torch.float32, (B, R)),
            "exact": v(lay.off_exact, B * R * 4, torch.float32, (B, R)),
            **({} if lay.flags & FPB_FLAG_APPROX_DIRECT else {
                "tau": v(lay.off_tau, B * Qp * 2, torch.float16, (B, Qp)),
                "hibits": v(lay.off_hibits, B * lay.hb_words * 4, torch.int32, (B, lay.hb_words)),
                "approx_lb": v(lay.off_lb, B * lay.cand_cap * 4, torch.float32, (B, lay.cand_cap)),
                "refine": v(lay.off_refine, B * lay.cand_cap * 4, torch.int32, (B, lay.cand_cap)),
            }),
            "n_refine": v(lay.off_n_refine, B * 4, torch.int32, (B,)),
            "thresh": v(lay.off_thresh, B * 4, torch.float32, (B,)),
            "stats": v(lay.off_stats, 64, torch.int64, (8,)),
        }

    def reconstruct(self, doc_ids: list[int]) -> list[torch.Tensor]:
        if not doc_ids:
            return []
        ids = torch.tensor(doc_ids, dtype=torch.int64)
        if int(ids.min()) < 0 or int(ids.max()) >= self.num_documents:
            raise ValueError("document id out of range")
        offs = self.doc_offsets.cpu()
        lens = offs[ids + 1] - offs[ids]
        out_off = torch.zeros(len(doc_ids) + 1, dtype=torch.int64)
        out_off[1:] = lens.cumsum(0)
        total = int(out_off[-1])
        out = torch.empty((max(total, 1), self.dim), dtype=torch.float16, device=self.device)
        d_ids = ids.to(self.device, torch.int32)
        d_off = out_off.to(self.device)
        with self._exclusive(), torch.cuda.device(self.device):
            _check(self._lib.fpb_reconstruct(self._handle, d_ids.data_ptr(), len(doc_ids), d_off.data_ptr(),
                                             out.data_ptr(), self._stream()))
        return [out[int(out_off[i]) : int(out_off[i + 1])] for i in range(len(doc_ids))]

    def token_scores(self, queries: torch.Tensor, query_of: torch.Tensor, doc_ids: torch.Tensor) -> torch.Tensor:
        queries = queries.contiguous()
        n = int(doc_ids.shape[0])
        Q = int(queries.shape[1])
        out = torch.zeros((max(n, 1), max(self.max_doc_len, 1), Q), dtype=torch.float16, device=self.device)
        if n == 0:
            return out[:0]
        qo = query_of.to(self.device, torch.int32).contiguous()
        di = doc_ids.to(self.device, torch.int32).contiguous()
        with self._exclusive(), torch.cuda.device(self.device):
            _check(self._lib.fpb_token_scores(self._handle, queries.data_ptr(), Q, qo.data_ptr(), di.data_ptr(), n,
                                              max(self.max_doc_len, 1), out.data_ptr(), self._stream()))
        return out
```

include/fastplaid_b200.h:

```cpp
#ifndef FASTPLAID_B200_H_
#define FASTPLAID_B200_H_

#include <stddef.h>
#include <stdint.h>

#ifdef __cplusplus
extern "C" {
#endif

#define FPB_OK 0
#define FPB_ERR_INVALID (-1)
#define FPB_ERR_CUDA (-2)
#define FPB_ERR_UNSUPPORTED (-3)
#define FPB_ERR_WORKSPACE (-4)
#define FPB_ERR_NO_IVF (-5)

typedef struct fpb_index fpb_index;
struct fpb_record;

const char* fpb_last_error(void);
int fpb_abi_version(void);

int fpb_index_create(fpb_index** out, int device, int nbits, int dim, int64_t n_centroids,
                     const void* d_centroids, const void* d_bucket_weights, int64_t n_docs,
                     const int64_t* d_doc_offsets, const int32_t* d_doc_codes,
                     const uint8_t* d_doc_residuals, void* d_token_norms, const int64_t* d_ivf_offsets,
                     const int32_t* d_ivf_pids, int64_t n_ivf, int64_t max_doc_len,
                     int64_t doc_id_base);
void fpb_index_destroy(fpb_index* index);

typedef struct fpb_params {
  int32_t n_ivf_probe;
  int32_t n_full_scores;
  int32_t top_k;
  int32_t batch_size;
  int32_t flags;
} fpb_params;

#define FPB_FLAG_SUBSET 1
#define FPB_FLAG_APPROX_EXACT_ALL 2
#define FPB_FLAG_APPROX_DIRECT 4
#define FPB_FLAG_APPROX_TWO_PASS 8

typedef struct fpb_layout {
  int64_t total_bytes;
  int32_t B, Q, Qp, n_tiles, R, n_probe, cand_cap, bitmap_words;
  int32_t cbitmap_words, reserved0;
  int64_t off_queries;
  int64_t off_S;
  int64_t off_tmax;
  int64_t off_cells;
  int64_t off_bitmap;
  int64_t off_n_cand;
  int64_t off_cand;
  int64_t off_approx;
  int64_t off_work;
  int64_t off_n_rerank;
  int64_t off_rerank;
  int64_t off_rerank_approx;
  int64_t off_exact;
  int64_t off_cbitmap;
  int64_t off_clist;
  int64_t off_n_clist;
  int64_t off_sbitmap;
  int64_t off_tau;
  int64_t off_hibits;
  int64_t off_lb;
  int64_t off_refine;
  int64_t off_n_refine;
  int64_t off_thresh;
  int64_t off_work2;
  int64_t off_stats;
  int32_t hb_words, flags;
} fpb_layout;

int fpb_workspace_layout(const fpb_index* index, int B, int Q, const fpb_params* params,
                         fpb_layout* out);

int fpb_search_batch(const fpb_index* index, const void* d_queries, int B, int Q,
                     const fpb_params* params, void* d_workspace, size_t workspace_bytes,
                     int64_t* d_out_ids, float* d_out_scores, int32_t* d_out_counts,
                     void* stream);

int fpb_search_batch_subset(const fpb_index* index, const void* d_queries, int B, int Q,
                            const fpb_params* params, const int32_t* d_subset_ids,
                            const int64_t* d_subset_offsets, int64_t max_subset_len, void* d_workspace,
                            size_t workspace_bytes, int64_t* d_out_ids, float* d_out_scores,
                            int32_t* d_out_counts, void* stream);

int fpb_search_batch_host(const fpb_index* index, const void* h_queries, int B, int Q,
                          const fpb_params* params, void* d_workspace, size_t workspace_bytes,
                          void* d_queries_staging, int64_t* d_out_ids, float* d_out_scores,
                          int32_t* d_out_counts, int64_t* h_out_ids, float* h_out_scores,
                          int32_t* h_out_counts, void* stream);

int fpb_stage_centroid_scores(const fpb_index*, const void* d_queries, int B, int Q,
                              const fpb_params*, void* d_workspace, size_t, void* stream);
int fpb_stage_subset(const fpb_index*, const int32_t* d_subset_ids, const int64_t* d_subset_offsets,
                     int64_t max_subset_len, int B, int Q, const fpb_params*, void* d_workspace, size_t,
                     void* stream);
int fpb_stage_probe(const fpb_index*, int B, int Q, const fpb_params*, void* d_workspace,
                    size_t, void* stream);
int fpb_stage_candidates(const fpb_index*, int B, int Q, const fpb_params*, void* d_workspace,
                         size_t, void* stream);
int fpb_stage_approx(const fpb_index*, int B, int Q, const fpb_params*, void* d_workspace,
                     size_t, void* stream);
int fpb_stage_select(const fpb_index*, int B, int Q, const fpb_params*, void* d_workspace,
                     size_t, void* stream);
int fpb_stage_maxsim(const fpb_index*, int B, int Q, const fpb_params*, void* d_workspace,
                     size_t, void* stream);
int fpb_stage_rank(const fpb_index*, int B, int Q, const fpb_params*, void* d_workspace,
                   size_t, int64_t* d_out_ids, float* d_out_scores, int32_t* d_out_counts,
                   void* stream);

int fpb_stage_keys(const fpb_index*, int B, int Q, const fpb_params*, void* d_workspace, size_t,
                   uint64_t* d_keys, void* stream);
int fpb_stage_records(const fpb_index*, int B, int Q, const fpb_params*, void* d_workspace, size_t,
                      struct fpb_record* d_records, void* stream);

struct fpb_record {
  float approx;
  float exact;
  int64_t doc_id;
};
typedef struct fpb_record fpb_record;

int fpb_search_shard(const fpb_index* index, const void* d_queries, int B, int Q,
                     const fpb_params* params, void* d_workspace, size_t workspace_bytes,
                     fpb_record* d_records , void* stream);
int fpb_merge_shards(const fpb_record* d_all_records , int n_shards,
                     int B, int R, int top_k, int64_t* d_out_ids, float* d_out_scores,
                     int32_t* d_out_counts, void* stream);

int fpb_shard_approx_keys(const fpb_index* index, const void* d_queries, int B, int Q,
                          const fpb_params* params, void* d_workspace, size_t workspace_bytes,
                          uint64_t* d_keys , void* stream);
int fpb_shard_subset_begin(const fpb_index* index, const void* d_queries, int B, int Q,
                           const fpb_params* params, const int32_t* d_subset_ids,
                           const int64_t* d_subset_offsets, int64_t max_subset_len, void* d_workspace,
                           size_t workspace_bytes, uint32_t* d_cbitmap_out, void* stream);
int fpb_shard_subset_keys(const fpb_index* index, int B, int Q, const fpb_params* params, void* d_workspace,
                          size_t workspace_bytes, const uint32_t* d_all_cbitmaps ,
                          int n_shards, uint64_t* d_keys , void* stream);
int fpb_shard_apply_threshold(const fpb_index* index, const uint64_t* d_all_keys ,
                              int n_shards, int shard_rank, int B, int Q, const fpb_params* params,
                              void* d_workspace, size_t workspace_bytes, void* stream);
int fpb_shard_exact_records(const fpb_index* index, int B, int Q, const fpb_params* params,
                            void* d_workspace, size_t workspace_bytes, fpb_record* d_records, void* stream);

#define FPB_COMM_ID_BYTES 128
typedef struct fpb_comm fpb_comm;
int fpb_comm_unique_id(void* out_id );
int fpb_comm_create(fpb_comm** out, int nranks, int rank, const void* unique_id, int device);
void fpb_comm_destroy(fpb_comm* comm);
int fpb_comm_nccl_version(void);
int64_t fpb_sharded_scratch_bytes(int b_local, int R, int nranks);
int fpb_search_batch_sharded(const fpb_index* index, fpb_comm* comm, int n_query_groups, const void* d_queries,
                             int B, int Q, const fpb_params* params, void* d_workspace, size_t workspace_bytes,
                             void* d_scratch, size_t scratch_bytes, int64_t* d_out_ids, float* d_out_scores,
                             int32_t* d_out_counts, void* stream);
int fpb_search_batch_sharded_host(const fpb_index* index, fpb_comm* comm, int n_query_groups, const void* h_queries,
                                  int B, int Q, const fpb_params* params, void* d_workspace, size_t workspace_bytes,
                                  void* d_scratch, size_t scratch_bytes, void* d_queries_staging, int64_t* d_out_ids,
                                  float* d_out_scores, int32_t* d_out_counts, int64_t* h_out_ids, float* h_out_scores,
                                  int32_t* h_out_counts, void* stream);

int fpb_exhaustive_workspace_bytes(const fpb_index* index, int B, int Q, int top_k, size_t* out);
int fpb_exhaustive_scores(const fpb_index* index, const void* d_queries, int B, int Q, void* d_workspace,
                          size_t workspace_bytes, float* d_scores, void* stream);
int fpb_search_exhaustive(const fpb_index* index, const void* d_queries, int B, int Q, int top_k, void* d_workspace,
                          size_t workspace_bytes, int64_t* d_out_ids, float* d_out_scores, int32_t* d_out_counts,
                          void* stream);

int fpb_reconstruct(const fpb_index* index, const int32_t* d_doc_ids, int n, const int64_t* d_out_offsets,
                    void* d_out, void* stream);
int fpb_token_scores(const fpb_index* index, const void* d_queries, int Q, const int32_t* d_query_of,
                     const int32_t* d_doc_ids, int n, int64_t max_len, void* d_out, void* stream);

int fpb_cast_f32_to_f16_host(const float* h_src, void* h_dst, size_t n);
int fpb_cast_f32_to_f16_host_portable(const float* h_src, void* h_dst, size_t n);

int fpb_encode(int device, int nbits, int dim, int64_t n_centroids, const void* d_centroids,
               const void* d_tokens, int64_t n_tokens, const float* d_cutoffs, int32_t* d_codes,
               uint8_t* d_residuals, void* stream);

int fpb_kmeans_assign(int device, int dim, int64_t n_centroids, const void* d_centroids, const float* d_bias,
                      const void* d_points, int64_t n_points, int32_t* d_assign, void* stream);
int fpb_kmeans_update(int device, int dim, int64_t n_centroids, const void* d_points, const int64_t* d_order,
                      const int64_t* d_seg_offsets, void* d_centroids, float* d_shift, void* stream);

#ifdef __cplusplus
}
#endif
#endif
```

Before: 2857.

## Precompute bank-sorted window-aligned code layout for approx and bound kernels

New measurement: 3143, median of 6. +10.0%, better.

```diff
diff --git a/fast_plaid_b200/csrc/common.cuh b/fast_plaid_b200/csrc/common.cuh
--- a/fast_plaid_b200/csrc/common.cuh
+++ b/fast_plaid_b200/csrc/common.cuh
@@ -27,6 +27,9 @@
   const int32_t* doc_codes;
   const uint8_t* doc_residuals;
   const __half* token_norms;
+  int32_t* walk_codes;
+  int64_t* walk_win;
+  int walk_group;
   const int64_t* ivf_offsets;
   const int32_t* ivf_pids;
   WPerm w_perm;
@@ -55,6 +58,10 @@
   } while (0)
 
 static inline int64_t fpb_align256(int64_t x) { return (x + 255) & ~int64_t(255); }
+static inline int fpb_hb_words(int64_t K) { return int(((K + 31) / 32 + 3) / 4 * 4); }
+__host__ __device__ inline int32_t fpb_walk_pad_code(int hb_words, int bank) {
+  return int32_t(hb_words + ((bank - hb_words) & 31)) * 32;
+}
 static inline int fpb_next_pow2(int x) {
   int p = 1;
   while (p < x) p <<= 1;
diff --git a/fast_plaid_b200/csrc/index.cu b/fast_plaid_b200/csrc/index.cu
--- a/fast_plaid_b200/csrc/index.cu
+++ b/fast_plaid_b200/csrc/index.cu
@@ -35,6 +35,44 @@
   return 0;
 }
 
+static int make_walk_layout(fpb_index* ix) {
+  const int64_t N = ix->N;
+  int64_t* offs = new int64_t[N + 1];
+  int64_t* win = new int64_t[N + 1];
+  offs[0] = 0;
+  cudaError_t e = N > 0 ? cudaMemcpy(offs, ix->doc_offsets, sizeof(int64_t) * (N + 1), cudaMemcpyDeviceToHost)
+                        : cudaSuccess;
+  win[0] = 0;
+  int64_t slots[3] = {0, 0, 0};
+  for (int64_t d = 0; d < N; ++d) {
+    const int64_t nw = (offs[d + 1] - offs[d] + 31) / 32;
+    win[d + 1] = win[d] + nw;
+    for (int g = 4; g <= 6; ++g) slots[g - 4] += (nw > g ? (nw + g - 1) / g : 1) * g;
+  }
+  ix->walk_group = 6;
+  for (int g = 5; g >= 4; --g)
+    if (slots[g - 4] < slots[ix->walk_group - 4]) ix->walk_group = g;
+  const int64_t n_win = win[N];
+  if (e == cudaSuccess) e = cudaMalloc(&ix->walk_win, sizeof(int64_t) * (N + 1));
+  if (e == cudaSuccess) e = cudaMemcpy(ix->walk_win, win, sizeof(int64_t) * (N + 1), cudaMemcpyHostToDevice);
+  if (e == cudaSuccess) e = cudaMalloc(&ix->walk_codes, sizeof(int32_t) * 32 * (n_win > 0 ? n_win : 1));
+  delete[] offs;
+  delete[] win;
+  if (e != cudaSuccess) {
+    fpb_set_error("walk layout: %s", cudaGetErrorString(e));
+    return FPB_ERR_CUDA;
+  }
+  if (n_win == 0) return FPB_OK;
+  const int rc = launch_walk_layout(ix, nullptr);
+  if (rc != FPB_OK) return rc;
+  e = cudaDeviceSynchronize();
+  if (e != cudaSuccess) {
+    fpb_set_error("walk layout kernel failed: %s", cudaGetErrorString(e));
+    return FPB_ERR_CUDA;
+  }
+  return FPB_OK;
+}
+
 static thread_local char g_err[512] = "";
 
 void fpb_set_error(const char* fmt, ...) {
@@ -78,7 +116,7 @@
     fpb_set_error("fpb_index_create: bad sizes or NULL codec/offset pointers");
     return FPB_ERR_INVALID;
   }
-  if (n_docs >= (int64_t(1) << 31) || n_centroids >= (int64_t(1) << 31)) {
+  if (n_docs >= (int64_t(1) << 31) || n_centroids >= (int64_t(1) << 31) - 2048) {
     fpb_set_error("fpb_index_create: n_docs and n_centroids must fit in int32 per shard");
     return FPB_ERR_UNSUPPORTED;
   }
@@ -142,12 +180,41 @@
       return rc != FPB_OK ? rc : FPB_ERR_CUDA;
     }
   }
+  const int rc = make_walk_layout(ix);
+  if (rc != FPB_OK) {
+    fpb_index_destroy(ix);
+    return rc;
+  }
   make_centroid_tmap(ix);
   *out = ix;
   return FPB_OK;
 }
 
-extern "C" void fpb_index_destroy(fpb_index* index) { delete index; }
+extern "C" void fpb_index_destroy(fpb_index* index) {
+  if (!index) return;
+  if (index->walk_codes || index->walk_win) {
+    int prev = -1;
+    const bool have_prev = cudaGetDevice(&prev) == cudaSuccess;
+    cudaSetDevice(index->device);
+    cudaFree(index->walk_codes);
+    cudaFree(index->walk_win);
+    if (have_prev) cudaSetDevice(prev);
+  }
+  delete index;
+}
+
+extern "C" int fpb_index_walk_layout(const fpb_index* ix, int64_t* n_windows, int32_t* d_codes, int64_t* d_win) {
+  if (!ix || !n_windows) {
+    fpb_set_error("fpb_index_walk_layout: NULL argument");
+    return FPB_ERR_INVALID;
+  }
+  FPB_CUDA_CHECK(cudaSetDevice(ix->device));
+  FPB_CUDA_CHECK(cudaMemcpy(n_windows, ix->walk_win + ix->N, sizeof(int64_t), cudaMemcpyDeviceToHost));
+  if (d_codes && *n_windows > 0)
+    FPB_CUDA_CHECK(cudaMemcpy(d_codes, ix->walk_codes, sizeof(int32_t) * 32 * *n_windows, cudaMemcpyDeviceToDevice));
+  if (d_win) FPB_CUDA_CHECK(cudaMemcpy(d_win, ix->walk_win, sizeof(int64_t) * (ix->N + 1), cudaMemcpyDeviceToDevice));
+  return FPB_OK;
+}
 
 extern "C" int fpb_workspace_layout(const fpb_index* ix, int B, int Q, const fpb_params* p,
                                     fpb_layout* L) {
@@ -214,7 +281,7 @@
   L->off_n_clist = take(sub ? int64_t(B) * 4 : 0);
   L->off_sbitmap = take(sub ? int64_t(B) * L->bitmap_words * 4 : 0);
   const bool direct = (p->flags & FPB_FLAG_APPROX_DIRECT) != 0;
-  L->hb_words = int(((ix->K + 31) / 32 + 3) / 4 * 4);
+  L->hb_words = fpb_hb_words(ix->K);
   L->off_tau = take(direct ? 0 : int64_t(B) * Qp * 2);
   L->off_hibits = take(direct ? 0 : int64_t(B) * L->hb_words * 4);
   L->off_lb = take(direct ? 0 : int64_t(B) * L->cand_cap * 4);
diff --git a/fast_plaid_b200/csrc/k3_approx.cu b/fast_plaid_b200/csrc/k3_approx.cu
--- a/fast_plaid_b200/csrc/k3_approx.cu
+++ b/fast_plaid_b200/csrc/k3_approx.cu
@@ -76,10 +76,77 @@
   return s;
 }
 
+constexpr int K3_WALK_THREADS = 256;
+
+__global__ void __launch_bounds__(K3_WALK_THREADS)
+k3_walk_layout_kernel(const int64_t* __restrict__ doc_offsets, const int32_t* __restrict__ codes,
+                      const int64_t* __restrict__ walk_win, int64_t N, int hb_words, int32_t* __restrict__ walk_codes) {
+  __shared__ int s_cnt[K3_WALK_THREADS / 32][32];
+  const int lane = threadIdx.x & 31, warp = threadIdx.x >> 5;
+  unsigned lt_mask;
+  asm("mov.u32 %0, %%lanemask_lt;" : "=r"(lt_mask));
+  int* cnt = s_cnt[warp];
+  for (int64_t d = int64_t(blockIdx.x) * (K3_WALK_THREADS / 32) + warp; d < N;
+       d += int64_t(gridDim.x) * (K3_WALK_THREADS / 32)) {
+    const int64_t o0 = doc_offsets[d];
+    const int len = int(doc_offsets[d + 1] - o0);
+    const int nw = (len + 31) >> 5;
+    int32_t* out = walk_codes + walk_win[d] * 32;
+    cnt[lane] = 0;
+    __syncwarp();
+    for (int t0 = 0; t0 < len; t0 += 32) {
+      const bool act = t0 + lane < len;
+      const unsigned am = __ballot_sync(0xffffffffu, act);
+      if (act) {
+        const int bank = (__ldg(codes + o0 + t0 + lane) >> 5) & 31;
+        const unsigned peers = __match_any_sync(am, bank);
+        if ((peers & lt_mask) == 0u) cnt[bank] += __popc(peers);
+      }
+      __syncwarp();
+    }
+    {
+      const int c = cnt[lane];
+      int incl = c;
+#pragma unroll
+      for (int off = 1; off < 32; off <<= 1) {
+        const int v = __shfl_up_sync(0xffffffffu, incl, off);
+        if (lane >= off) incl += v;
+      }
+      __syncwarp();
+      cnt[lane] = incl - c;
+      __syncwarp();
+    }
+    for (int t0 = 0; t0 < len; t0 += 32) {
+      const bool act = t0 + lane < len;
+      const unsigned am = __ballot_sync(0xffffffffu, act);
+      int code = 0, bank = 0, i = 0;
+      unsigned peers = 0u;
+      if (act) {
+        code = __ldg(codes + o0 + t0 + lane);
+        bank = (code >> 5) & 31;
+        peers = __match_any_sync(am, bank);
+        i = cnt[bank] + __popc(peers & lt_mask);
+      }
+      __syncwarp();
+      if (act && (peers & lt_mask) == 0u) cnt[bank] += __popc(peers);
+      __syncwarp();
+      if (act) out[(i % nw) * 32 + i / nw] = code;
+    }
+    __syncwarp();
+    for (int w = 0; w < nw; ++w) {
+      const int r = (len - w + nw - 1) / nw;
+      const unsigned used = __reduce_or_sync(0xffffffffu, lane < r ? 1u << ((out[w * 32 + lane] >> 5) & 31) : 0u);
+      if (lane >= r) out[w * 32 + lane] = fpb_walk_pad_code(hb_words, int(__fns(~used, 0, lane - r + 1)));
+    }
+    __syncwarp();
+  }
+}
+
 template <int LPR, int UNROLL, int MINB>
 __global__ void __launch_bounds__(K3_THREADS, MINB)
 k3_approx_kernel(const __half* __restrict__ S, int64_t K, int Q, const int64_t* __restrict__ doc_offsets,
-                 const int32_t* __restrict__ codes, const int32_t* __restrict__ cand, int cand_cap,
+                 const int32_t* __restrict__ walk_codes, const int64_t* __restrict__ walk_win,
+                 const int32_t* __restrict__ cand, int cand_cap,
                  const int32_t* __restrict__ n_cand, const int32_t* __restrict__ list,
                  const int32_t* __restrict__ n_list, int32_t* __restrict__ work, int B,
                  float* __restrict__ approx, unsigned long long* __restrict__ stats) {
@@ -88,6 +155,7 @@
   __shared__ int s_b, s_c;
   const int tid = threadIdx.x, lane = tid & 31, warp = tid >> 5;
   const int sub = lane % LPR, grp = lane / LPR;
+  const int Ki = int(K);
   const __half2 sentinel = __float2half2_rn(FPB_PAD_SENTINEL);
   unsigned long long rows = 0;
 
@@ -109,20 +177,19 @@
       const int64_t o0 = doc_offsets[d];
       const int len = int(doc_offsets[d + 1] - o0);
       rows += unsigned(len);
+      const int nw = (len + 31) >> 5;
+      const int32_t* cw = walk_codes + walk_win[d] * 32 + lane;
       __half2 m0 = sentinel, m1 = sentinel, m2 = sentinel, m3 = sentinel;
-      for (int base = 0; base < len; base += 32 * UNROLL) {
+      for (int w0 = 0; w0 < nw; w0 += UNROLL) {
         int code[UNROLL];
 #pragma unroll
-        for (int u = 0; u < UNROLL; ++u) {
-          const int t = base + u * 32 + lane;
-          code[u] = (t < len) ? __ldg(codes + o0 + t) : -1;
-        }
+        for (int u = 0; u < UNROLL; ++u) code[u] = (w0 + u < nw) ? __ldg(cw + (w0 + u) * 32) : Ki;
 #pragma unroll
         for (int u = 0; u < UNROLL; ++u) {
 #pragma unroll
           for (int jj = 0; jj < LPR; ++jj) {
             const int c = __shfl_sync(0xffffffffu, code[u], jj * TPI + grp);
-            if (c >= 0) {
+            if (c < Ki) {
               const uint4 v = __ldg(Sb + int64_t(c) * LPR + sub);
               m0 = __hmax2(m0, u32_as_half2(v.x));
               m1 = __hmax2(m1, u32_as_half2(v.y));
@@ -157,14 +224,16 @@
 template <int LPR, int UNROLL, int MINB>
 __global__ void __launch_bounds__(K3_THREADS, MINB)
 k3_approx_nsh_kernel(const __half* __restrict__ S, int64_t K, int Q, const int64_t* __restrict__ doc_offsets,
-                     const int32_t* __restrict__ codes, int64_t n_codes, const int32_t* __restrict__ cand,
-                     int cand_cap, const int32_t* __restrict__ n_cand, const int32_t* __restrict__ list,
-                     const int32_t* __restrict__ n_list, int32_t* __restrict__ work, int B,
-                     float* __restrict__ approx, unsigned long long* __restrict__ stats) {
+                     const int32_t* __restrict__ walk_codes, const int64_t* __restrict__ walk_win,
+                     const int32_t* __restrict__ cand, int cand_cap, const int32_t* __restrict__ n_cand,
+                     const int32_t* __restrict__ list, const int32_t* __restrict__ n_list,
+                     int32_t* __restrict__ work, int B, float* __restrict__ approx,
+                     unsigned long long* __restrict__ stats) {
   constexpr int QP = LPR * 8;
   __shared__ int s_b, s_c;
   const int tid = threadIdx.x, lane = tid & 31, warp = tid >> 5;
   const int sub = lane % LPR, grp = lane / LPR;
+  const int Ki = int(K);
   const __half2 sentinel = __float2half2_rn(FPB_PAD_SENTINEL);
   unsigned long long rows = 0;
 
@@ -186,29 +255,25 @@
       const int64_t o0 = doc_offsets[d];
       const int len = int(doc_offsets[d + 1] - o0);
       rows += unsigned(len);
-      const int64_t w0 = o0 & ~int64_t(31);
-      const int lo = int(o0 - w0), hi = lo + len;
-      const int32_t* cw = codes + w0 + grp * LPR;
-      const int64_t readable = n_codes - (w0 + grp * LPR);
+      const int nw = (len + 31) >> 5;
+      const int32_t* cw = walk_codes + walk_win[d] * 32 + grp * LPR;
       __half2 m0 = sentinel, m1 = sentinel, m2 = sentinel, m3 = sentinel;
-      for (int f0 = 0; f0 < hi; f0 += 32 * UNROLL) {
+      for (int w0 = 0; w0 < nw; w0 += UNROLL) {
         int c[UNROLL][LPR];
 #pragma unroll
         for (int u = 0; u < UNROLL; ++u) {
-          const int fo = f0 + u * 32;
-          if (fo + LPR <= readable) {
-            load_codes<LPR>(c[u], cw + fo);
+          if (w0 + u < nw) {
+            load_codes<LPR>(c[u], cw + (w0 + u) * 32);
           } else {
 #pragma unroll
-            for (int jj = 0; jj < LPR; ++jj) c[u][jj] = (fo + jj < readable) ? __ldg(cw + fo + jj) : 0;
+            for (int jj = 0; jj < LPR; ++jj) c[u][jj] = Ki;
           }
         }
 #pragma unroll
         for (int u = 0; u < UNROLL; ++u) {
 #pragma unroll
           for (int jj = 0; jj < LPR; ++jj) {
-            const int f = f0 + u * 32 + grp * LPR + jj;
-            if (unsigned(f - lo) < unsigned(len)) {
+            if (c[u][jj] < Ki) {
               const uint4 v = __ldg(Sb + int64_t(c[u][jj]) * LPR);
               m0 = __hmax2(m0, u32_as_half2(v.x));
               m1 = __hmax2(m1, u32_as_half2(v.y));
@@ -232,7 +297,8 @@
 template <int LPR>
 __global__ void __launch_bounds__(K3_TAU_THREADS)
 k3_tau_kernel(const __half* __restrict__ S, int64_t K, int Q, const int64_t* __restrict__ doc_offsets,
-              const int32_t* __restrict__ codes, const int32_t* __restrict__ cand, int cand_cap,
+              const int32_t* __restrict__ walk_codes, const int64_t* __restrict__ walk_win,
+              const int32_t* __restrict__ cand, int cand_cap,
               const int32_t* __restrict__ n_cand, const __half* __restrict__ tmax, int n_tiles, float lambda,
               __half* __restrict__ tau) {
   constexpr int QP = LPR * 8, TPI = 32 / LPR;
@@ -243,6 +309,7 @@
   __shared__ int s_redo;
   const int b = blockIdx.x, tid = threadIdx.x, lane = tid & 31, warp = tid >> 5;
   const int sub = lane % LPR, grp = lane / LPR;
+  const int Ki = int(K);
   uint16_t* out = reinterpret_cast<uint16_t*>(tau) + int64_t(b) * QP;
   const int n = n_cand[b];
   const int ns = min(n, K3_TAU_DOCS);
@@ -275,11 +342,10 @@
       for (int e = 0; e < 8; ++e) fl[e] = (mine && !s_redo) ? s_floor[qrow + e] : 0u;
       for (int j = warp; j < ns; j += K3_TAU_THREADS / 32) {
         const int d = cb[int64_t(j) * n / ns];
-        const int64_t o0 = doc_offsets[d];
-        const int len = int(doc_offsets[d + 1] - o0);
-        for (int base = 0; base < len; base += 32) {
-          const int t = base + lane;
-          const int code = (t < len) ? __ldg(codes + o0 + t) : -1;
+        const int nw = int((doc_offsets[d + 1] - doc_offsets[d] + 31) >> 5);
+        const int32_t* cw = walk_codes + walk_win[d] * 32 + lane;
+        for (int w = 0; w < nw; ++w) {
+          const int code = __ldg(cw + w * 32);
           constexpr int JB = LPR < 8 ? LPR : 8;
 #pragma unroll 1
           for (int j0 = 0; j0 < LPR; j0 += JB) {
@@ -289,12 +355,12 @@
           for (int jj = 0; jj < JB; ++jj) {
             cc[jj] = __shfl_sync(0xffffffffu, code, (j0 + jj) * TPI + grp);
             vv[jj] = make_uint4(0u, 0u, 0u, 0u);
-            if (cc[jj] >= 0 && mine) vv[jj] = __ldg(Sb + int64_t(cc[jj]) * LPR + sub);
+            if (cc[jj] < Ki && mine) vv[jj] = __ldg(Sb + int64_t(cc[jj]) * LPR + sub);
           }
 #pragma unroll
           for (int jj = 0; jj < JB; ++jj) {
             const int c = cc[jj];
-            if (c >= 0 && mine) {
+            if (c < Ki && mine) {
               const uint4 v = vv[jj];
               const uint32_t w[4] = {v.x, v.y, v.z, v.w};
 #pragma unroll
@@ -413,7 +479,8 @@
 template <int LPR, int MINB, int W, int U, bool FULLQ, bool PAIR>
 __global__ void __launch_bounds__(K3_THREADS, MINB)
 k3_bound_kernel(const __half* __restrict__ S, int64_t K, int Q, const int64_t* __restrict__ doc_offsets,
-                const int32_t* __restrict__ codes, const int32_t* __restrict__ cand, int cand_cap,
+                const int32_t* __restrict__ walk_codes, const int64_t* __restrict__ walk_win,
+                const int32_t* __restrict__ cand, int cand_cap,
                 const int32_t* __restrict__ n_cand, int32_t* __restrict__ work, int B,
                 const __half* __restrict__ tau, const uint32_t* __restrict__ hibits, int hb_words,
                 float* __restrict__ ub_out, float* __restrict__ lb_out, unsigned long long* __restrict__ stats) {
@@ -425,19 +492,19 @@
   static_assert(FLUSH + 32 * W <= WQ, "ring too small");
   extern __shared__ __align__(16) uint32_t k3_smem[];
   __shared__ int s_b, s_c;
-  __shared__ int64_t s_o0[K3A_DOCS_PER_CHUNK];
+  __shared__ int64_t s_w0[K3A_DOCS_PER_CHUNK];
   __shared__ int s_len[K3A_DOCS_PER_CHUNK];
   const int tid = threadIdx.x, lane = tid & 31, warp = tid >> 5;
   const int sub = lane % LPR, grp = lane / LPR;
   const uint32_t sb_bm = smem_u32(k3_smem);
-  const uint32_t sb_wq = ((sb_bm + uint32_t(hb_words + 4) * 4u + (WQ * 4u - 1u)) & ~(WQ * 4u - 1u)) + uint32_t(warp) * (WQ * 4u);
+  const uint32_t sb_wq = ((sb_bm + uint32_t(hb_words + 32) * 4u + (WQ * 4u - 1u)) & ~(WQ * 4u - 1u)) + uint32_t(warp) * (WQ * 4u);
   const int INV = hb_words * 32;
   unsigned lt_mask;
   asm("mov.u32 %0, %%lanemask_lt;" : "=r"(lt_mask));
   const __half2 sentinel = __float2half2_rn(FPB_PAD_SENTINEL);
   unsigned rows = 0, toks = 0;
   int cur_b = -1;
-  if (tid < 4) k3_smem[hb_words + tid] = 0u;
+  if (tid < 32) k3_smem[hb_words + tid] = 0u;
 
   for (;;) {
     k3_next_chunk(work, B, &s_b, &s_c);
@@ -447,14 +514,14 @@
     const int32_t* cb = cand + int64_t(b) * cand_cap;
     if (tid < K3A_DOCS_PER_CHUNK) {
       const int idx = s_c * K3A_DOCS_PER_CHUNK + tid;
-      int64_t o0 = 0;
+      int64_t w0 = 0;
       int len = -1;
       if (idx < n) {
         const int d = cb[idx];
-        o0 = doc_offsets[d];
-        len = int(doc_offsets[d + 1] - o0);
-      }
-      s_o0[tid] = o0;
+        w0 = walk_win[d];
+        len = int(doc_offsets[d + 1] - doc_offsets[d]);
+      }
+      s_w0[tid] = w0;
       s_len[tid] = len;
     }
     if (b != cur_b) {
@@ -472,20 +539,13 @@
     const int slot_end = slot + DPW;
     int len = s_len[slot];
     if (len < 0) continue;
-    int rel, left;
-    const int32_t* cw;
-    {
-      const int64_t o0 = s_o0[slot];
-      const int lo = int(o0 & 31);
-      rel = lane - lo;
-      left = (lo + len + 31) >> 5;
-      cw = codes + (o0 - lo) + lane;
-    }
+    int left = (len + 31) >> 5;
+    const int32_t* cw = walk_codes + s_w0[slot] * 32 + lane;
     int c[W];
 #pragma unroll
     for (int u = 0; u < W; ++u) {
       c[u] = INV;
-      if (unsigned(rel + 32 * u) < unsigned(len)) c[u] = __ldg(cw + 32 * u);
+      if (u < left) c[u] = __ldg(cw + 32 * u);
     }
     uint32_t head = 0, tail = 0;
     __half2 m0 = sentinel, m1 = sentinel, m2 = sentinel, m3 = sentinel;
@@ -494,26 +554,21 @@
 
     for (;;) {
       const bool last_of_doc = left <= W;
-      int nlen = len, nrel = rel + 32 * W, nleft = left - W;
+      int nlen = len, nleft = left - W;
       const int32_t* ncw = cw + 32 * W;
       if (last_of_doc) {
         nlen = (slot + 1 < slot_end) ? s_len[slot + 1] : -1;
+        nleft = 0;
         if (nlen >= 0) {
-          const int64_t o0 = s_o0[slot + 1];
-          const int lo = int(o0 & 31);
-          nrel = lane - lo;
-          nleft = (lo + nlen + 31) >> 5;
-          ncw = codes + (o0 - lo) + lane;
+          nleft = (nlen + 31) >> 5;
+          ncw = walk_codes + s_w0[slot + 1] * 32 + lane;
         }
       }
       int nx[W];
-      {
-        const unsigned nlen_u = nlen < 0 ? 0u : unsigned(nlen);
-#pragma unroll
-        for (int u = 0; u < W; ++u) {
-          nx[u] = INV;
-          if (unsigned(nrel + 32 * u) < nlen_u) nx[u] = __ldg(ncw + 32 * u);
-        }
+#pragma unroll
+      for (int u = 0; u < W; ++u) {
+        nx[u] = INV;
+        if (u < nleft) nx[u] = __ldg(ncw + 32 * u);
       }
       uint32_t wbit[W];
 #pragma unroll
@@ -614,7 +669,6 @@
 #pragma unroll
       for (int u = 0; u < W; ++u) c[u] = nx[u];
       len = nlen;
-      rel = nrel;
       left = nleft;
       cw = ncw;
     }
@@ -1055,28 +1109,44 @@
   const fpb_layout& L = *ws.L;
   const int blocks = ix->sm_count * 8;
   if constexpr (LPR <= 4) {
-    if ((reinterpret_cast<uintptr_t>(ix->doc_codes) & 15u) == 0) {
-      k3_approx_nsh_kernel<LPR, 2, 6><<<blocks, K3_THREADS, 0, st>>>(
-          ws.S(), ix->K, L.Q, ix->doc_offsets, ix->doc_codes, ix->E, ws.cand(), L.cand_cap, ws.n_cand(), list, n_list,
-          work, L.B, ws.approx(), ws.stats());
-      FPB_LAUNCH_CHECK("k3_approx_nsh");
-      return FPB_OK;
-    }
-  }
-  k3_approx_kernel<LPR, 2, 6><<<blocks, K3_THREADS, 0, st>>>(ws.S(), ix->K, L.Q, ix->doc_offsets, ix->doc_codes,
-                                                             ws.cand(), L.cand_cap, ws.n_cand(), list, n_list, work,
-                                                             L.B, ws.approx(), ws.stats());
+    k3_approx_nsh_kernel<LPR, 2, 6><<<blocks, K3_THREADS, 0, st>>>(
+        ws.S(), ix->K, L.Q, ix->doc_offsets, ix->walk_codes, ix->walk_win, ws.cand(), L.cand_cap, ws.n_cand(), list,
+        n_list, work, L.B, ws.approx(), ws.stats());
+    FPB_LAUNCH_CHECK("k3_approx_nsh");
+    return FPB_OK;
+  }
+  k3_approx_kernel<LPR, 2, 6><<<blocks, K3_THREADS, 0, st>>>(ws.S(), ix->K, L.Q, ix->doc_offsets, ix->walk_codes,
+                                                             ix->walk_win, ws.cand(), L.cand_cap, ws.n_cand(), list,
+                                                             n_list, work, L.B, ws.approx(), ws.stats());
   FPB_LAUNCH_CHECK("k3_approx");
   return FPB_OK;
 }
 
 float k3_tau_lambda(int Q) {
-  static const float pinned = [] {
-    const char* e = getenv("FPB_K3_LAMBDA");
-    return e ? float(atof(e)) : 0.f;
-  }();
+  const char* e = getenv("FPB_K3_LAMBDA");
+  const float pinned = e ? float(atof(e)) : 0.f;
   const float x = pinned > 0.f ? pinned : logf(float(Q < 2 ? 2 : Q)) - 1.45f;
   return x < 0.5f ? 0.5f : (x > 64.f ? 64.f : x);
+}
+
+template <int LPR, int W>
+int launch_k3_bound(const fpb_index* ix, const Ws& ws, cudaStream_t st) {
+  const fpb_layout& L = *ws.L;
+  constexpr int TPI = 32 / LPR;
+  constexpr int U = 4, MINB = 4;
+  const bool fullq = L.Q == L.Qp;
+  auto kern = fullq ? k3_bound_kernel<LPR, MINB, W, U, true, true> : k3_bound_kernel<LPR, MINB, W, U, false, true>;
+  const int minb = MINB, wq = K3_WQ_FOR(W, U * TPI);
+  const size_t smem = size_t(L.hb_words + 32) * 4 + size_t(K3_THREADS / 32 + 1) * wq * 4;
+  FPB_CUDA_CHECK(cudaFuncSetAttribute(kern, cudaFuncAttributeMaxDynamicSharedMemorySize, int(smem)));
+  int per_sm = int((227 * 1024) / (smem + 1024 + 2048));
+  per_sm = per_sm < 1 ? 1 : (per_sm > minb ? minb : per_sm);
+  kern<<<ix->sm_count * per_sm, K3_THREADS, smem, st>>>(ws.S(), ix->K, L.Q, ix->doc_offsets, ix->walk_codes,
+                                                        ix->walk_win, ws.cand(), L.cand_cap, ws.n_cand(), ws.work(),
+                                                        L.B, ws.tau(), ws.hibits(), L.hb_words, ws.approx(), ws.lb(),
+                                                        ws.stats());
+  FPB_LAUNCH_CHECK("k3_bound");
+  return FPB_OK;
 }
 
 template <int LPR>
@@ -1090,9 +1160,9 @@
     FPB_LAUNCH_CHECK("k3_prefix");
     return launch_k3_exact<LPR>(ix, ws, nullptr, nullptr, ws.work(), st);
   }
-  k3_tau_kernel<LPR><<<L.B, K3_TAU_THREADS, 0, st>>>(ws.S(), ix->K, L.Q, ix->doc_offsets, ix->doc_codes, ws.cand(),
-                                                     L.cand_cap, ws.n_cand(), ws.tmax(), L.n_tiles, k3_tau_lambda(L.Q),
-                                                     ws.tau());
+  k3_tau_kernel<LPR><<<L.B, K3_TAU_THREADS, 0, st>>>(ws.S(), ix->K, L.Q, ix->doc_offsets, ix->walk_codes,
+                                                     ix->walk_win, ws.cand(), L.cand_cap, ws.n_cand(), ws.tmax(),
+                                                     L.n_tiles, k3_tau_lambda(L.Q), ws.tau());
   FPB_LAUNCH_CHECK("k3_tau");
   {
     dim3 grid(unsigned((ix->K + 255) / 256), unsigned(L.B));
@@ -1102,19 +1172,11 @@
   k3_prefix_kernel<<<1, 32, 0, st>>>(ws.n_cand(), L.B, K3A_DOCS_PER_CHUNK, ws.work());
   FPB_LAUNCH_CHECK("k3_prefix");
   {
-    constexpr int TPI = 32 / LPR;
-    constexpr int W = 6, U = 4, MINB = 4;
-    const bool fullq = L.Q == L.Qp;
-    auto kern = fullq ? k3_bound_kernel<LPR, MINB, W, U, true, true> : k3_bound_kernel<LPR, MINB, W, U, false, true>;
-    const int minb = MINB, wq = K3_WQ_FOR(W, U * TPI);
-    const size_t smem = size_t(L.hb_words + 4) * 4 + size_t(K3_THREADS / 32 + 1) * wq * 4;
-    FPB_CUDA_CHECK(cudaFuncSetAttribute(kern, cudaFuncAttributeMaxDynamicSharedMemorySize, int(smem)));
-    int per_sm = int((227 * 1024) / (smem + 1024 + 2048));
-    per_sm = per_sm < 1 ? 1 : (per_sm > minb ? minb : per_sm);
-    kern<<<ix->sm_count * per_sm, K3_THREADS, smem, st>>>(ws.S(), ix->K, L.Q, ix->doc_offsets, ix->doc_codes, ws.cand(),
-                                                          L.cand_cap, ws.n_cand(), ws.work(), L.B, ws.tau(),
-                                                          ws.hibits(), L.hb_words, ws.approx(), ws.lb(), ws.stats());
-    FPB_LAUNCH_CHECK("k3_bound");
+    const char* e = getenv("FPB_K3_GROUP");
+    const int g = e ? atoi(e) : ix->walk_group;
+    const int rc = g == 4 ? launch_k3_bound<LPR, 4>(ix, ws, st)
+                 : g == 5 ? launch_k3_bound<LPR, 5>(ix, ws, st) : launch_k3_bound<LPR, 6>(ix, ws, st);
+    if (rc != FPB_OK) return rc;
   }
   k3_refine_list_kernel<<<L.B, 1024, 0, st>>>(ws.approx(), ws.lb(), L.cand_cap, ws.n_cand(), L.R,
                                               (flags & FPB_FLAG_APPROX_EXACT_ALL) ? 1 : 0, ws.refine(), ws.n_refine(),
@@ -1141,6 +1203,17 @@
   }
 }
 
+int launch_walk_layout(const fpb_index* ix, cudaStream_t st) {
+  if (ix->N == 0) return FPB_OK;
+  const int64_t warps = K3_WALK_THREADS / 32;
+  const int64_t need = (ix->N + warps - 1) / warps;
+  const int blocks = int(need < int64_t(ix->sm_count) * 16 ? need : int64_t(ix->sm_count) * 16);
+  k3_walk_layout_kernel<<<blocks, K3_WALK_THREADS, 0, st>>>(ix->doc_offsets, ix->doc_codes, ix->walk_win, ix->N,
+                                                            fpb_hb_words(ix->K), ix->walk_codes);
+  FPB_LAUNCH_CHECK("k3_walk_layout");
+  return FPB_OK;
+}
+
 int launch_select(const fpb_index* ix, const Ws& ws, cudaStream_t st) {
   (void)ix;
   const fpb_layout& L = *ws.L;
diff --git a/fast_plaid_b200/csrc/kernels.h b/fast_plaid_b200/csrc/kernels.h
--- a/fast_plaid_b200/csrc/kernels.h
+++ b/fast_plaid_b200/csrc/kernels.h
@@ -45,6 +45,7 @@
 int launch_compact(const uint32_t* bitmap, const uint32_t* mask, int words, int32_t* out, int cap, int32_t* n_out,
                    int B, cudaStream_t st);
 int launch_approx(const fpb_index* ix, const Ws& ws, int flags, cudaStream_t st);
+int launch_walk_layout(const fpb_index* ix, cudaStream_t st);
 int launch_select(const fpb_index* ix, const Ws& ws, cudaStream_t st);
 int launch_maxsim(const fpb_index* ix, const Ws& ws, cudaStream_t st);
 int launch_token_norms(const fpb_index* ix, __half* d_out, cudaStream_t st);
diff --git a/fast_plaid_b200/engine.py b/fast_plaid_b200/engine.py
--- a/fast_plaid_b200/engine.py
+++ b/fast_plaid_b200/engine.py
@@ -90,6 +90,7 @@
     "fpb_abi_version",
     "fpb_index_create",
     "fpb_index_destroy",
+    "fpb_index_walk_layout",
     "fpb_workspace_layout",
     "fpb_search_batch",
     "fpb_search_batch_subset",
@@ -156,6 +157,8 @@
         ]
         lib.fpb_index_destroy.restype = None
         lib.fpb_index_destroy.argtypes = [vp]
+        lib.fpb_index_walk_layout.restype = i32
+        lib.fpb_index_walk_layout.argtypes = [vp, ctypes.POINTER(i64), vp, vp]
         lib.fpb_workspace_layout.restype = i32
         lib.fpb_workspace_layout.argtypes = [vp, i32, i32, ctypes.POINTER(FpbParams), ctypes.POINTER(FpbLayout)]
         lib.fpb_search_batch.restype = i32
@@ -1020,6 +1023,15 @@
             "stats": v(lay.off_stats, 64, torch.int64, (8,)),
         }
 
+    def walk_layout(self) -> tuple[torch.Tensor, torch.Tensor]:
+        n = ctypes.c_int64()
+        with self._exclusive(), torch.cuda.device(self.device):
+            _check(self._lib.fpb_index_walk_layout(self._handle, ctypes.byref(n), None, None))
+            codes = torch.empty((max(n.value, 1), 32), dtype=torch.int32, device=self.device)
+            win = torch.empty(self.num_documents + 1, dtype=torch.int64, device=self.device)
+            _check(self._lib.fpb_index_walk_layout(self._handle, ctypes.byref(n), codes.data_ptr(), win.data_ptr()))
+        return codes[: n.value], win
+
     def reconstruct(self, doc_ids: list[int]) -> list[torch.Tensor]:
         if not doc_ids:
             return []
diff --git a/include/fastplaid_b200.h b/include/fastplaid_b200.h
--- a/include/fastplaid_b200.h
+++ b/include/fastplaid_b200.h
@@ -28,6 +28,7 @@
                      const int32_t* d_ivf_pids, int64_t n_ivf, int64_t max_doc_len,
                      int64_t doc_id_base);
 void fpb_index_destroy(fpb_index* index);
+int fpb_index_walk_layout(const fpb_index* index, int64_t* n_windows, int32_t* d_codes, int64_t* d_win);
 
 typedef struct fpb_params {
   int32_t n_ivf_probe;
```
